# YuliangXiu/ICON

Hardware: AMD Instinct MI355X
Metric: query-points/sec at 256^3 grid (higher is better)
Workload: dtype f32 via 3x f16 split MFMA (22-bit operands, f32 accumulate)

## Files before the change

icon_amd/_lib.py:

```python
from __future__ import annotations

import ctypes as C
import os
import subprocess

_HERE = os.path.dirname(os.path.abspath(__file__))
LIB_PATH = os.environ.get("ICON_AMD_LIB") or os.path.join(_HERE, "libicon_amd.so")
CSRC = os.path.join(_HERE, "csrc")

PRIOR = {"icon": 0, "pamir": 1, "pifu": 2}
CMAP = {"reference": 0, "local": 1}
SEARCH = {"bvh": 0, "brute": 1}
PRECISION = {"f32": 0, "f16x3": 1}

SYMBOLS = [
    "icon_last_error", "icon_version", "icon_device_count",
    "icon_mesh_create", "icon_mesh_destroy", "icon_mesh_vertex_normals", "icon_mesh_stats",
    "icon_mesh_arena_bytes", "icon_mesh_create_arena", "icon_mesh_status", "icon_debug_set_mesh_build", "icon_debug_mesh_layout", "icon_debug_host_mesh_build",
    "icon_sdf_query",
    "icon_feat_create", "icon_feat_destroy", "icon_feat_set_smpl_feats",
    "icon_mlp_create", "icon_mlp_destroy", "icon_mlp_forward", "icon_mlp_set_last_op",
    "icon_work_create", "icon_work_destroy", "icon_work_profile", "icon_work_stage_ms", "icon_work_profile_detail", "icon_work_profile_workgroups", "icon_work_set_steal", "icon_work_set_reserve_cus",
    "icon_query_points", "icon_query_points_dcalib", "icon_query_rows", "icon_grid_rows",
    "icon_volume_any_above", "icon_adaptive_eval", "icon_adaptive_counts", "icon_adaptive_reruns", "icon_grid_eval_slab", "icon_grid_slab_features", "icon_grid_slab_finish", "icon_grid_slab_features_msg",
    "icon_grid_slab_finish_gathered", "icon_debug_set_shell_skip", "icon_debug_set_option", "icon_work_status", "icon_sdf_query_ties", "icon_work_set_tie_rule",
    "icon_export_mesh", "icon_mc_count", "icon_mc_emit", "icon_mc_count_range", "icon_mc_emit_keyed", "icon_debug_traversal_stats", "icon_debug_pair_stats", "icon_debug_walk_stats", "icon_debug_pair_box", "icon_debug_range_box", "icon_debug_box_bound", "icon_debug_box_bound_half", "icon_debug_set_unfused", "icon_debug_mlp_pack_f16x3",
    "icon_visibility", "icon_mesh_components", "icon_clean_mesh", "icon_semantic_voxelize",
    "icon_mesh_batch_create", "icon_mesh_batch_destroy", "icon_mesh_batch_status", "icon_feat_create_batch", "icon_query_points_batch",
    "icon_feat_batch_set_volume", "icon_semantic_voxelize_batch",
    "icon_query_color_bytes", "icon_query_color",
    "icon_render_bytes", "icon_render_normal",
    "icon_silhouette_bytes", "icon_silhouette_forward", "icon_silhouette_backward",
    "icon_render_normal_backward_bytes", "icon_render_normal_backward",
    "icon_render_turntable_bytes", "icon_render_turntable",
    "icon_local_affine_bytes", "icon_local_affine_forward", "icon_local_affine_backward",
    "icon_mesh_priors_bytes", "icon_mesh_priors_forward", "icon_mesh_priors_backward",
    "icon_smpl_bytes", "icon_smpl_forward", "icon_smpl_backward",
    "icon_nearest_vertex", "icon_extract_cloth_bytes", "icon_extract_cloth",
    "icon_normal_consistency_bytes", "icon_normal_consistency",
    "icon_sample_geo_bytes", "icon_sample_geo",
    "icon_train_rows_bytes", "icon_train_rows_forward", "icon_train_rows_backward",
    "icon_train_pamir_forward", "icon_train_vol_bytes", "icon_train_vol_backward",
]

_lib = None


class IconAmdError(RuntimeError):
    pass


def build(force: bool = False) -> str:
    args = ["make", "-j8", "-C", CSRC] + (["-B"] if force else [])
    proc = subprocess.run(args, stdout=subprocess.PIPE, stderr=subprocess.STDOUT, text=True)
    if proc.returncode != 0:
        raise IconAmdError("building libicon_amd.so failed:\n" + proc.stdout[-4000:])
    return LIB_PATH


def lib():
    global _lib
    if _lib is not None:
        return _lib
    if not os.path.exists(LIB_PATH):
        raise IconAmdError(f"{LIB_PATH} not found - run `python -c 'import __graft_entry__ as g; g.build()'` "
                           "or `make -C icon_amd/csrc` (needs hipcc); there is no CPU fallback")
    import torch
    L = C.CDLL(LIB_PATH)
    L.icon_last_error.restype = C.c_char_p
    for name in SYMBOLS:
        if name != "icon_last_error":
            getattr(L, name).restype = C.c_int
    _lib = L
    return L


def check(rc: int, what: str = "") -> None:
    if rc != 0:
        msg = lib().icon_last_error().decode("utf-8", "replace")
        raise IconAmdError(f"{what or 'icon_amd'} failed (code {rc}): {msg}")


def device_count() -> int:
    return int(lib().icon_device_count())


def require_device() -> None:
    if device_count() < 1:
        raise IconAmdError("icon_amd needs a HIP device (MI355X); none is visible and there is no CPU fallback")


def ptr(t) -> C.c_void_p:
    if t is None:
        return C.c_void_p(0)
    if hasattr(t, "data_ptr"):
        assert t.is_contiguous(), "tensor must be contiguous"
        return C.c_void_p(t.data_ptr())
    return C.c_void_p(t.ctypes.data)
```

icon_amd/csrc/common.h:

```cpp
#pragma once
#include <hip/hip_runtime.h>
#include <stdint.h>
#include <functional>
#include <string>
#include <vector>

#include "../../include/icon_amd.h"

namespace icon {
constexpr int kWgRec = 6;
constexpr int kMaxProfGrid = 1024;

void set_error(const std::string &msg);
int fail(int code, const std::string &msg);

#define ICON_HIP(expr)                                                                          \
    do {                                                                                        \
        hipError_t _e = (expr);                                                                 \
        if (_e != hipSuccess)                                                                   \
            return ::icon::fail(ICON_ERR_HIP, std::string(#expr) + ": " + hipGetErrorString(_e)); \
    } while (0)

#define ICON_ARG(cond, msg)                                                  \
    do {                                                                     \
// ... 146 lines not shown
    const float wx[2] = {(float)x1 - ix, ix - (float)t.x0};
    const float wy[2] = {(float)y1 - iy, iy - (float)t.y0};
    const float wz[2] = {(float)z1 - iz, iz - (float)t.z0};
    const bool bx[2] = {t.x0 >= 0 && t.x0 < W, x1 >= 0 && x1 < W};
    const bool by[2] = {t.y0 >= 0 && t.y0 < H, y1 >= 0 && y1 < H};
    const bool bz[2] = {t.z0 >= 0 && t.z0 < D, z1 >= 0 && z1 < D};
#pragma unroll
    for (int k = 0; k < 8; ++k) {
        t.w[k] = (wx[k & 1] * wy[(k >> 1) & 1]) * wz[k >> 2];
        t.in[k] = bx[k & 1] && by[(k >> 1) & 1] && bz[k >> 2];
    }
    t.any = (bx[0] || bx[1]) && (by[0] || by[1]) && (bz[0] || bz[1]);
    return t;
}
__device__ __forceinline__ float trilinear_sample(const TrilinearTaps &t, const float *__restrict__ vol, int H, int W)
{
    float acc = 0.0f;
#pragma unroll
    for (int k = 0; k < 8; ++k) {
        const float v = t.in[k] ? vol[((int64_t)(t.z0 + (k >> 2)) * H + (t.y0 + ((k >> 1) & 1))) * W + (t.x0 + (k & 1))] : 0.0f;
        const float prod = v * t.w[k];
        acc = k == 0 ? prod : acc + prod;
    }
    return acc;
}

struct Calib { float m[12]; const float *d; };

struct Lattice {
    int32_t res, z0, z1;
};

struct LatticeMap {
    int res, z0, nz;
    int tx, ty, tz;
    int remap;
    int off;
    int zs, nzi;
    int sx0, sx1, sy0, sy1;
    int sz0, sz1;
    int trim;
    float trim_need;
    int pk;
};

__device__ __forceinline__ bool not_finite(float y)
{
    uint32_t u = __float_as_uint(y);
    asm volatile("" : "+v"(u));
    return (u & 0x7f800000u) == 0x7f800000u;
}

__device__ __forceinline__ float apply_last_op(float y, int last_op)
{
    return last_op == ICON_LASTOP_SIGMOID ? 1.0f / (1.0f + expf(-y)) : y;
}

struct NearRef { uint16_t *lo; uint8_t *hi; float *d2; const int32_t *map; };

struct SignSrc;

struct BatchDev {
    const MeshDev *meshes;
    const float *calibs;
    int64_t n;
    int64_t plane_stride;
    int B;
    int64_t vol_stride;
};
enum class Src { Lattice, Points, Batch };

}

struct icon_mesh {
    int64_t V = 0, F = 0;
    char *arena = nullptr;
    size_t arena_bytes = 0;
    bool owns_arena = false;
    float *d_vnormals = nullptr;
    icon::MeshDyn *d_dyn = nullptr;
    icon::MeshDyn *h_dyn = nullptr;
    hipEvent_t built = nullptr;
    int depth_bound = 0;
    icon::MeshDev dev{};
};

struct icon_feat {
    float *d_planes = nullptr;
    float *d_vol = nullptr;
    icon::FeatDev dev{};
    int batch = 1;
    int64_t plane_stride = 0;
    int64_t vol_stride = 0;
};

struct icon_mesh_batch {
    int B = 0;
    int64_t V = 0, F = 0;
    int depth_bound = 0;
    std::vector<const icon_mesh *> subj;
    icon::MeshDev *d_table = nullptr;
    icon::MeshDev *h_table = nullptr;
    int *h_status = nullptr;
    hipEvent_t done = nullptr;
};

struct icon_adaptive;
struct icon_mlp {
    int c0 = 0;
    int last_op = 0;
    float *d_blob = nullptr;
    size_t blob_bytes = 0;
    size_t off_w0 = 0, off_b0 = 0, off_w1 = 0, off_b1 = 0, off_w2 = 0, off_w2x = 0, off_b2 = 0, off_w3 = 0;
    size_t off_plain = 0;
    size_t off_flag = 0;
    float b3 = 0.f;
    char *d_f16 = nullptr;
    float f16_inv[3] = {1.f, 1.f, 1.f};
};

namespace icon {
void parallel_for(int n, const std::function<void(int)> &fn);
void debug_sync(const char *what, hipStream_t st);
struct MeshLayout;
int mesh_host_state_get(MeshDyn **h, hipEvent_t *ev);
void mesh_host_state_put(MeshDyn *h, hipEvent_t ev);
void mesh_bind_arena(icon_mesh *m, const MeshLayout &L);
int mesh_build_device(icon_mesh *m, const float *d_verts, const int64_t *d_faces, const float *d_cmap, const float *d_vis, hipStream_t st);
void adaptive_destroy(icon_adaptive *a);
inline int lattice_packet()
{
    static const int pk_env = getenv("ICON_AMD_PACKET") ? atoi(getenv("ICON_AMD_PACKET")) : 0;
    return pk_env == 2 ? 2 : 4;
}
struct McDevState;
void mc_destroy(McDevState *s);
struct CleanState;
void clean_destroy(CleanState *s);
int morton_order(icon_work *w, const float *d_points, const float *calib12, const float *d_calib12, int64_t N, hipStream_t st, const int32_t **perm);
int mlp_launch(const icon_mlp *mlp, const float *d_x, int64_t N, float *d_out, int precision, hipStream_t st);
int mlp_launch_ex(const icon_mlp *mlp, const float *d_x, int64_t N, float *d_out, bool mask, hipStream_t st);
int mlp_rescue_rows(const icon_mlp *mlp, const float *d_x, int64_t N, float *d_out, hipStream_t st);
int mlp_flag_reset(const icon_mlp *mlp, hipStream_t st);
int rescue_always();
int mlp_pack_f16x3(icon_mlp *m, const std::vector<std::vector<float>> &W, const std::vector<std::vector<float>> &B, hipStream_t st);
int mlp_launch_f16x3(const icon_mlp *mlp, const float *d_x, int64_t N, float *d_out, bool mask, hipStream_t st);
uint16_t f32_to_f16_rtn(float f);
float f16_to_f32(uint16_t h);
float pick_scale(const std::vector<float> &W);
int morton_order_batch(icon_work *w, const float *d_points, const float *d_calibs, int64_t n, int B, hipStream_t st, const int32_t **perm);
int ensure_work(icon_work *w, int64_t n_points, bool need_x);
void mark(icon_work *w, int k, hipStream_t st);
bool want_fused(int precision, int search);
int outlier_list(icon_work *w, int64_t N, const int *n_dev, int8_t *signs, bool counted, hipStream_t st);
SignSrc self_signs(const icon_work *work, bool needs);
int resolve_signs(const icon_work *work, SignSrc *sg, hipStream_t st);
int outlier_patch(icon_work *w, int64_t N, int cmap_slot, const SignSrc &sg, hipStream_t st);
int pack_sign_message(const icon_work *w, const int8_t *signs, void *d_msg, int64_t cap, hipStream_t st);
int device_cu_count(int *n_cu);
int once_per_device(int kernel_id, const std::function<hipError_t()> &set);
struct LatticeFast;
struct ShareDbg {
    int *err;
    int ring, lose, spin_log2;
};
int work_share_dbg(icon_work *w, ShareDbg *out);
int work_check_err(icon_work *w);
extern int g_qc_lanes;
extern int g_rn_lanes;
extern int g_tt_chunk;
extern int g_ev_lanes;
enum Opt { kOptPairBox, kOptNodeBox, kOptBoxClamp, kOptLatticeFast, kOptUnfused, kOptShellSkip, kOptMcClassify1, kOptShareWaves, kOptShareRing, kOptShareLose,
           kOptShareSpinLog2, kOptCount };
int option(Opt o);
}

namespace icon {
constexpr float kIdentCalib[12] = {1, 0, 0, 0, 0, 1, 0, 0, 0, 0, 1, 0};
constexpr int kNearLoSlots = 32768;

struct QueryCall {
    const char *who = "";
    Src src = Src::Points;
    const icon_mesh *mesh = nullptr;
    const icon_mesh_batch *mb = nullptr;
    BatchDev bd{};
    const icon_feat *feat = nullptr;
    int prior = 0, cmap_mode = 0, search = 0;
    float sdf_clip = 0.f;
    Calib cal{};
    LatticeMap L{};
    const float *points = nullptr;
    int64_t N = 0;
    const int32_t *map = nullptr;
    const int *n_dev = nullptr;
    int c0 = 0;
    int cmap_slot = 0;
    bool needs_patch = false;
    bool rows_ready = false, patched = false;
};
inline QueryCall query_call(const char *who, Src src, const icon_feat *feat, int prior, float sdf_clip, int cmap_mode, int search)
{
    QueryCall c;
    c.who = who; c.src = src; c.feat = feat; c.prior = prior; c.sdf_clip = sdf_clip; c.cmap_mode = cmap_mode; c.search = search;
    return c;
}
int describe_call(QueryCall &c);
int describe_call(QueryCall &c, const FeatDev &f);
bool coop_search(int64_t N, const icon_work *work);
int call_geometry(QueryCall &c, int8_t *d_signs_out, icon_work *work, hipStream_t st);
int sign_and_list(const QueryCall &c, int8_t *d_signs_out, icon_work *work, hipStream_t st);
int call_finish(QueryCall &c, const icon_mlp *mlp, const SignSrc &fs, float *d_occ, int precision, icon_work *work, hipStream_t st, int za = 0, int zb = 0);
int launch_nearest_batch(const QueryCall &c, icon_work *work, hipStream_t st);
int launch_sign(const QueryCall &c, const icon_work *work, hipStream_t st);
int launch_fused_f16x3(const QueryCall &c, const icon_mlp *mlp, const icon_work *work, int za, int zb, const SignSrc &fs, float *d_occ, hipStream_t st);
int begin_call(icon_work *w, const QueryCall &c, bool need_x = false);
}

struct icon_work {
    float *d_x = nullptr;
    int64_t cap_x = 0;
    uint16_t *d_near16 = nullptr;
    uint8_t *d_near_hi = nullptr;
    float *d_near_d2 = nullptr;
    int64_t cap_points_hi = 0;
    uint8_t *d_code8 = nullptr;
    int64_t cap_points = 0;
    uint64_t *d_grp_mask = nullptr;
    int32_t *d_block_counts = nullptr;
    int64_t *d_block_offsets = nullptr;
    int32_t *d_scan_local = nullptr;
    int64_t *d_scan_part = nullptr;
    int64_t cap_blocks = 0;
    int8_t *d_signs = nullptr;
    int64_t cap_signs = 0;
    int64_t *d_total = nullptr;
    int *d_flag = nullptr;
    mutable bool flag_clean = false;
    int64_t *d_seg = nullptr;
    int32_t *d_row_count = nullptr;
    int32_t *d_row_slots = nullptr;
    int64_t cap_rows = 0;
    int *h_err = nullptr;
    icon::LatticeFast *d_lfast = nullptr;
    uint32_t *d_sort_keys = nullptr;
    int32_t *d_sort_idx = nullptr;
    void *d_sort_tmp = nullptr;
    size_t sort_tmp_bytes = 0;
    int64_t cap_sort = 0;
    icon::QueryCall slab{};
    bool slab_ready = false;
    int tie_rule = 0, tie_ulps = 0;
    int reserve_cus = 0;
    int *h_any = nullptr;
    int *defer_range_flag = nullptr;
    int range_reruns = 0;
    struct icon_adaptive *ad = nullptr;
    icon::McDevState *mc = nullptr;
    icon::CleanState *clean = nullptr;
    bool prof = false;
    hipEvent_t ev[6] = {nullptr, nullptr, nullptr, nullptr, nullptr, nullptr};
    bool ev_search = false;
    unsigned long long *d_clock = nullptr;
    mutable int clock_grid = 0;
    double clock_kernel_ms = 0.0;
    unsigned int *d_steal = nullptr;
    int steal_permille = 150, steal_grp = 2;
    bool ev_valid = false;
};

namespace icon {
inline NearRef work_near(const icon_work *w, const QueryCall &c)
{
    NearRef r;
    r.lo = w->d_near16; r.d2 = w->d_near_d2;
    r.hi = (c.mesh && c.mesh->F > kNearLoSlots) ? w->d_near_hi : nullptr;
    r.map = c.map;
    return r;
}
}
```

icon_amd/csrc/fused_f16x3.hip:

```cpp
#pragma clang fp contract(off)

#include "geom_device.h"
#include "batch_device.h"
#include "mlp_f16x3_device.h"
#include "mlp_plain_device.h"
#include "sign_list_device.h"

#include <algorithm>
#include <mutex>

namespace icon {

constexpr int kTilePts = kF16Pts;
constexpr int kXsOff = kSideOff + 4352;
constexpr int kFusedLds = kXsOff + kTilePts * kXRow * 4;

struct FusedGeom {
    MeshDev m;
    FeatDev f;
    Calib cal;
    int res, z0;
    int off, nx, zs;
    uint32_t nx_magic;
    const float *pts;
    int64_t N;
    const int *n_dev;
    const int32_t *out_map;
    float sdf_clip;
    int cmap_local;
    NearRef near;
    const uint8_t *code8;
    const int64_t *block_offsets;
    const unsigned long long *grp_mask;
    SignSrc sg;
    unsigned long long *clock;
    unsigned int *steal;
    int steal_static, steal_grp, steal_ngrp;
};
constexpr int kPoolOff = kSideOff + kSideFloats * 4;
enum { kPoolNext = 0, kPoolMask, kPoolDone, kPoolPer, kPoolRem, kPoolStatic, kPoolGroup, kPoolNGrp, kPoolGrid, kPoolWords };
static_assert(kPoolOff + 4 * kPoolWords <= kSideOff + 4352, "the draw state lives in the slack behind the side arrays");
constexpr int kPoolLenShift = 24;
constexpr int kMaxStealGroup = 127;

__device__ __forceinline__ void pool_draw(unsigned int *steal, volatile int *pool)
{
    unsigned xcc;
    asm volatile("s_getreg_b32 %0, hwreg(HW_REG_XCC_ID)" : "=s"(xcc));
    const int per = pool[kPoolPer], rem = pool[kPoolRem], stat = pool[kPoolStatic], grp = pool[kPoolGroup], ngrp = pool[kPoolNGrp],
              grid = pool[kPoolGrid];
    int mask = pool[kPoolMask], word = -1;
    for (int s = 0; s < 8 && word < 0; ++s) {
        const int x = (int)((xcc + (unsigned)s) & 7u);
        if ((mask >> x) & 1) continue;
        const int nwg = (grid - x + 7) >> 3;
        for (;;) {
            const int t = (int)atomicAdd(steal + x, 1u);
            if (t >= nwg * ngrp) { mask |= 1 << x; break; }
            const int k = t / ngrp, g = t - k * ngrp, b = x + 8 * k;
            const int sb = b * per + min(b, rem), eb = sb + per + (b < rem ? 1 : 0);
            const int a = sb + stat + g * grp;
            if (a < eb) { word = a | (min(grp, eb - a) << kPoolLenShift); break; }
        }
    }
    pool[kPoolMask] = mask;
    pool[kPoolNext] = word;
}

__device__ __forceinline__ void wg_stamp(unsigned long long *rec)
{
    rec[0] = __builtin_readcyclecounter();
    rec[1] = __builtin_amdgcn_s_memrealtime();
}

static_assert(kScanBlock == 256, "k_sign's 256-point blocks are the blocks of the outlier scan and the tiles of the fused kernel");
template <bool LATTICE>
__global__ __launch_bounds__(256) void k_sign(MeshDev m, Calib cal, int res, int z0, const float *__restrict__ pts, int64_t N,
                                              float sdf_clip, const int32_t *__restrict__ row_count, const int32_t *__restrict__ row_slots,
                                              NearRef near, uint8_t *__restrict__ code8,
                                              int32_t *__restrict__ block_counts, unsigned long long *__restrict__ grp_mask, float far_box2,
                                              const int *__restrict__ n_dev, int *__restrict__ range_flag)
{
    __shared__ int wsum[4];
    if (range_flag && blockIdx.x == 0 && threadIdx.x == 0) *range_flag = 0;
    if (n_dev) { N = *n_dev; if ((int64_t)blockIdx.x * 256 >= N) return; }
    const int64_t i = (int64_t)blockIdx.x * 256 + threadIdx.x;
    const bool live = i < N;
    uint32_t code = 0;
    if (live) {
    f3 p; bool ins;
    if (LATTICE) {
        const int64_t row = i / res;
        const int ix = (int)(i - row * res), iy = (int)(row % res), iz = (int)(row / res);
        p = lattice_world(res, ix, iy, iz + z0);
        ins = inside_row(m, p, row_count, row_slots, row);
    } else {
        p = project(resolve_calib(cal), mk3(pts[3 * i], pts[3 * i + 1], pts[3 * i + 2]));
        ins = inside_bins(m, p);
    }
    const MeshDyn &d = *m.dyn;
    const bool far = box_dist2(d.box_lo[0], d.box_lo[1], d.box_lo[2], d.box_hi[0], d.box_hi[1], d.box_hi[2], p) > far_box2 || near_is_far(near, i);
    code = far ? sign_code_far(p, ins) : sign_code(p, near_d2(near, i), ins, sdf_clip);
    code8[i] = (uint8_t)code;
    }
    const unsigned long long b = __ballot(live && (code & kCodeOutlier));
    if ((threadIdx.x & 63) == 0) {
        wsum[threadIdx.x >> 6] = __popcll(b);
        grp_mask[(int64_t)blockIdx.x * 4 + (threadIdx.x >> 6)] = b;
    }
    __syncthreads();
    if (threadIdx.x == 0) block_counts[blockIdx.x] = wsum[0] + wsum[1] + wsum[2] + wsum[3];
}

template <bool BATCH>
__global__ __launch_bounds__(1024) void k_sign_wide(MeshDev m, Calib cal, const float *__restrict__ pts, int64_t N, float sdf_clip, NearRef near,
                                                    uint8_t *__restrict__ code8, int32_t *__restrict__ block_counts,
                                                    unsigned long long *__restrict__ grp_mask, float far_box2, const int *__restrict__ n_dev,
                                                    int *__restrict__ range_flag, BatchDev bd)
{
    __shared__ unsigned long long gm[4];
    if (range_flag && blockIdx.x == 0 && threadIdx.x == 0) *range_flag = 0;
    if (!BATCH && n_dev) { N = *n_dev; if ((int64_t)blockIdx.x * 256 >= N) return; }
    if (threadIdx.x < 4) gm[threadIdx.x] = 0ull;
    __syncthreads();
    const int s = threadIdx.x & 3, pt = threadIdx.x >> 2;
    const int64_t i = (int64_t)blockIdx.x * 256 + pt;
    const bool live = i < N;
    if (BATCH) {
        const int64_t b = (live ? i : N - 1) / bd.n;
        m = bd.meshes[b]; cal = batch_calib(bd, b);
    }
    uint32_t code = 0;
    const MeshDyn &d = *m.dyn;
    f3 p = mk3(0.f, 0.f, 0.f);
    int beg = 0, end = 0;
    bool brute = false;
    if (live) {
        p = project(resolve_calib(cal), mk3(pts[3 * i], pts[3 * i + 1], pts[3 * i + 2]));
        if (d.gy == 0) brute = true;
        else if (p.y >= d.bin_y0 && p.y <= d.bin_y1 && p.z >= d.bin_z0 && p.z <= d.bin_z1) {
            const int cy = bin_cell(p.y, d.bin_y0, d.bin_inv_y, d.gy);
            const int cz = bin_cell(p.z, d.bin_z0, d.bin_inv_z, d.gz);
            const int cell = cz * d.gy + cy;
            beg = m.bin_start[cell]; end = m.bin_start[cell + 1];
        }
    }
    int cnt = 0;
    for (int k = beg + s; k < end; k += 4) {
        f3 a, b, c; int ia, ib, ic;
        load_tri_full(m.tris + m.bin_slots[k], a, b, c, ia, ib, ic);
        cnt += ray_hit(p, a, b, c, ia, ib, ic);
    }
    cnt += __shfl_xor(cnt, 1);
    cnt += __shfl_xor(cnt, 2);
    if (live) {
        const bool ins = brute ? inside_brute(m, p) : ((cnt & 1) != 0);
        const bool far = box_dist2(d.box_lo[0], d.box_lo[1], d.box_lo[2], d.box_hi[0], d.box_hi[1], d.box_hi[2], p) > far_box2 || near_is_far(near, i);
        code = far ? sign_code_far(p, ins) : sign_code(p, near_d2(near, i), ins, sdf_clip);
        if (s == 0) code8[i] = (uint8_t)code;
    }
    unsigned long long x = __ballot(live && s == 0 && (code & kCodeOutlier));
    x = (x | (x >> 3)) & 0x0303030303030303ull;
    x = (x | (x >> 6)) & 0x000f000f000f000full;
    x = (x | (x >> 12)) & 0x000000ff000000ffull;
    x = (x | (x >> 24)) & 0xffffull;
    const int wave = threadIdx.x >> 6;
    if ((threadIdx.x & 63) == 0 && x) atomicOr(&gm[wave >> 2], x << (16 * (wave & 3)));
    __syncthreads();
    if (threadIdx.x < 4) grp_mask[(int64_t)blockIdx.x * 4 + threadIdx.x] = gm[threadIdx.x];
    if (threadIdx.x == 0) block_counts[blockIdx.x] = __popcll(gm[0]) + __popcll(gm[1]) + __popcll(gm[2]) + __popcll(gm[3]);
}

__global__ __launch_bounds__(256) void k_shell_zero(float *__restrict__ out, int res, int z0, int za, int zb, int row_wgs)
{
    const int planes = zb - za;
    if ((int)blockIdx.x < row_wgs) {
        const int64_t row = (int64_t)blockIdx.x * 256 + threadIdx.x;
        if (row >= (int64_t)planes * res) return;
        const int iy = (int)(row % res), iz = za + (int)(row / res);
        float *o = out + ((int64_t)(iz - z0) * res + iy) * res;
        o[0] = 0.0f; o[res - 1] = 0.0f;
        return;
    }
    const int f = ((int)blockIdx.x - row_wgs) * 4 + (int)(threadIdx.x >> 6);
    const int lane = threadIdx.x & 63;
    int iy, iz;
    if (f < 2 * planes) { iz = za + (f >> 1); iy = (f & 1) ? res - 1 : 0; }
    else {
        const int g = f - 2 * planes;
        const bool has0 = za == 0, has1 = zb == res;
        const int pl = g / res;
        if (pl >= (has0 ? 1 : 0) + (has1 ? 1 : 0)) return;
        iz = (pl == 0 && has0) ? 0 : res - 1;
        iy = g % res;
    }
    float *o = out + ((int64_t)(iz - z0) * res + iy) * res;
    for (int x = lane; x < res; x += 64) o[x] = 0.0f;
}

__device__ __forceinline__ int64_t lattice_item(const FusedGeom &G, int64_t q, int &ix, int &iy, int &iz)
{
    const uint32_t nx = (uint32_t)G.nx, qq = (uint32_t)q;
    const uint32_t r = udiv_fast(qq, nx, G.nx_magic), lx = qq - r * nx, lz = udiv_fast(r, nx, G.nx_magic), ly = r - lz * nx;
    ix = G.off + (int)lx; iy = G.off + (int)ly; iz = G.zs + (int)lz;
    return ((int64_t)(iz - G.z0) * G.res + iy) * G.res + ix;
}

__device__ __forceinline__ int64_t uniform64(int64_t v)
{
    const uint32_t lo = (uint32_t)__builtin_amdgcn_readfirstlane((int)(uint32_t)v);
    const uint32_t hi = (uint32_t)__builtin_amdgcn_readfirstlane((int)(uint32_t)((uint64_t)v >> 32));
    return (int64_t)(((uint64_t)hi << 32) | lo);
}

__device__ __forceinline__ void icon_row(const FusedGeom &G, const MeshDev &m, const FeatDev &f, f3 p, int64_t i, float *xrow, int64_t K, int64_t rank0)
{
    const uint32_t code = G.code8[i];
    Nearest nr;
    nr.slot = near_slot_of(G.near, i); nr.face = 0;
    nr.d2 = (code & kCodeOutlier) ? 0.0f : near_d2(G.near, i);
    const SdfOut o = sdf_attrs(m, p, nr, (code & kCodeInside) != 0);
    float s = o.sdf;
    f3 cmv = o.cm;
    if (code & kCodeOutlier) {
        s = (float)code_sign(code);
        if (G.cmap_local) cmv = mk3(s, s, s);
        else if (K > 0 && (f.smpl_mask & kSmplCmap)) {
            const int64_t blk = i >> 8;
            const int g = (int)(i >> 6) & 3;
            const unsigned long long *mk = G.grp_mask + blk * 4;
            int before = __popcll(mk[g] & ((1ull << (i & 63)) - 1ull));
            if (g > 0) before += __popcll(mk[0]);
            if (g > 1) before += __popcll(mk[1]);
            if (g > 2) before += __popcll(mk[2]);
            const int64_t jr = rank0 + G.block_offsets[blk] + before;
            float c3[3];
            outlier_cmap(G.sg, K, jr, c3);
            cmv = mk3(c3[0], c3[1], c3[2]);
        }
    }
    gather_planes_dyn(f, (f.n_select == 2 && o.vis == 0.0f) ? 1 : 0, p.x, p.y, xrow);
    int hh = f.csel;
    xrow[hh++] = s;
    if (f.smpl_mask & kSmplCmap) { xrow[hh] = cmv.x; xrow[hh + 1] = cmv.y; xrow[hh + 2] = cmv.z; hh += 3; }
    if (f.smpl_mask & kSmplNorm) { xrow[hh] = o.nrm.x; xrow[hh + 1] = o.nrm.y; xrow[hh + 2] = o.nrm.z; }
    xrow[kCodeSlot] = __int_as_float((int)(code & kCodeInCube));
}

template <int PRIOR, Src SRC>
__device__ __forceinline__ void build_row(const FusedGeom &G, const BatchDev &bd, int64_t q, float *xrow, int64_t K, int64_t rank0)
{
    f3 p;
    int64_t i;
    const int64_t b = SRC == Src::Batch ? q / bd.n : 0;
    if (SRC == Src::Lattice) {
        int ix, iy, iz;
        i = lattice_item(G, q, ix, iy, iz);
        p = lattice_world(G.res, ix, iy, iz);
    } else {
        i = q;
        p = project(SRC == Src::Batch ? batch_calib(bd, b) : resolve_calib(G.cal), mk3(G.pts[3 * i], G.pts[3 * i + 1], G.pts[3 * i + 2]));
    }
    const FeatDev f = SRC == Src::Batch ? batch_feat(G.f, bd, b) : G.f;
    if (PRIOR == ICON_PRIOR_ICON) {
// ... 54 lines not shown
            pool[kPoolPer] = per; pool[kPoolRem] = rem; pool[kPoolStatic] = G.steal_static; pool[kPoolGroup] = G.steal_grp;
            pool[kPoolNGrp] = G.steal_ngrp; pool[kPoolGrid] = (int)gridDim.x; pool[kPoolDone] = 0; pool[kPoolMask] = 0; pool[kPoolNext] = -1;
            if (stealing && tile >= tile_end) pool_draw(G.steal, pool);
        }
        __syncthreads();
        if (stealing && tile >= tile_end) {
            const int word = __builtin_amdgcn_readfirstlane(pool[kPoolNext]);
            __syncthreads();
            if (word >= 0) { tile = word & ((1 << kPoolLenShift) - 1); tile_end = tile + (word >> kPoolLenShift); }
        }
    }
    if (tile < tile_end) issue_chunk(w.image, smem, 0, wave0, lane0);

    for (int nb = -1; tile < tile_end;) {
        int tid = threadIdx.x;
        asm volatile("" : "+v"(tid));
        const int lane = tid & 63, wave = __builtin_amdgcn_readfirstlane(tid >> 6);
        const int r = lane & 15, g = lane >> 4;
        const int t = tid;
        const bool draw = !SMALL && stealing && tile + 1 == tile_end;
        if (!SMALL && draw && t == 256) pool_draw(G.steal, pool);
        const bool worker = t < tp;
        int64_t q = (int64_t)tile * tp + (worker ? t : 0);
        if (q >= G.N) q = G.N - 1;
        if (worker) build_row<PRIOR, SRC>(G, bd, q, Xs + t * kXRow, K, rank0);
        __syncthreads();

        nb = (!SMALL && draw) ? __builtin_amdgcn_readfirstlane(pool[kPoolNext]) : -1;
        if (!SMALL && tid == 0) pool[kPoolDone] = pool[kPoolDone] + 1;
        const bool more = tile + 1 < tile_end || nb >= 0;
        if (SMALL && wave >= (tp >> 5)) {
#pragma nounroll
            for (int c = 0; c < 14; c += 2) {
                issue_chunk_units<32>(w.image, smem + kBufBytes, c + 1, wave, lane);
                ICON_CHUNK_BARRIER();
                issue_chunk_units<32>(w.image, smem, c + 2, wave, lane);
                ICON_CHUNK_BARRIER();
            }
            issue_chunk_units<32>(w.image, smem + kBufBytes, 15, wave, lane);
            ICON_CHUNK_BARRIER();
            issue_chunk_units<40>(w.image, smem, 16, wave, lane);
            ICON_CHUNK_BARRIER();
            issue_chunk_units<32>(w.image, smem + kBufBytes, 17, wave, lane);
            ICON_CHUNK_BARRIER();
            issue_chunk_units<32>(w.image, smem, 18, wave, lane);
            ICON_CHUNK_BARRIER();
            issue_chunk_units<32>(w.image, smem + kBufBytes, 19, wave, lane);
            ICON_CHUNK_BARRIER();
            if (more) issue_chunk_units<32>(w.image, smem, 0, wave, lane);
            ++tile;
            continue;
        }
        const int pt = wave * 32 + 16 * (g & 1) + r;
        half8 xb[2];
        const float tail = load_x(Xs + (wave * 32 + r) * kXRow + 8 * (g & 1), Xs + (wave * 32 + 16 + r) * kXRow + 8 * (g & 1), sw3, w.c0, g, xb);
        float maskf = (__float_as_int(Xs[pt * kXRow + kCodeSlot]) & (int)kCodeInCube) ? 1.0f : 0.0f;
        asm volatile("" : "+v"(maskf));

        f32x4 acc1[16][2];
#pragma unroll
        for (int m = 0; m < 16; ++m) acc1[m][0] = acc1[m][1] = *reinterpret_cast<const f32x4 *>(sb1 + m * 16 + 4 * g);
        half8 bh[2], bl[2];
        const LeakyK k0{w.inv0, w.p0, w.q0}, k1{w.inv1, w.p1, w.q1};
        f32x4 acc2[8][2];
        layer01(smem, sb0, w.image, acc1, xb, k0, g, lane, wave, bh, bl);
#pragma unroll
        for (int m2 = 0; m2 < 8; ++m2) acc2[m2][0] = acc2[m2][1] = *reinterpret_cast<const f32x4 *>(sb2 + m2 * 16 + 4 * g);
        activate_split(acc1[0][0], acc1[1][0], acc1[0][1], acc1[1][1], k1, bh, bl);
        l2_chunk<0>(smem, smem + kBufBytes, w.image, acc1, acc2, xb, k1, g, lane, wave, bh, bl);
        ICON_CHUNK_BARRIER();
        l2_chunk<1>(smem + kBufBytes, smem, w.image, acc1, acc2, xb, k1, g, lane, wave, bh, bl);
        ICON_CHUNK_BARRIER();
        l2_chunk<2>(smem, smem + kBufBytes, w.image, acc1, acc2, xb, k1, g, lane, wave, bh, bl);
        ICON_CHUNK_BARRIER();
        l2_chunk<3>(smem + kBufBytes, smem, w.image, acc1, acc2, xb, k1, g, lane, wave, bh, bl, more);

        float y2[2];
        {
            int tid_3 = threadIdx.x;
            asm volatile("" : "+v"(tid_3), "+v"(acc2[0][0]));
            l3_sum(sw3, acc2, tail, LeakyK{w.inv2, w.p2, w.q2}, w.b3, (tid_3 >> 4) & 3, y2);
        }
        int tid_o = threadIdx.x;
        asm volatile("" : "+v"(tid_o), "+v"(y2[0]), "+v"(y2[1]));
        const int g_o = (tid_o >> 4) & 3, pt_o = (tid_o >> 6) * 32 + 16 * (g_o & 1) + (tid_o & 15);
        const float y = apply_last_op(g_o == 0 ? y2[0] : y2[1], w.last_op);
        const int64_t oq = (int64_t)tile * tp + pt_o;
        if (g_o < 2 && oq < G.N) {
            int ix, iy, iz;
            out[SRC == Src::Lattice ? lattice_item(G, oq, ix, iy, iz) : ((SRC == Src::Points && G.out_map) ? (int64_t)G.out_map[oq] : oq)] = masked_result(y, maskf != 0.0f, w.flag);
        }
        if (!SMALL && nb >= 0) {
            tile = nb & ((1 << kPoolLenShift) - 1);
            tile_end = tile + (nb >> kPoolLenShift);
        } else ++tile;
    }
    if (!SMALL && stealing && threadIdx.x == 0) {
        __threadfence();
        if (atomicAdd(G.steal + 8, 1u) == gridDim.x - 1)
            for (int k = 0; k < 9; ++k) atomicExch(G.steal + k, 0u);
    }
    if (G.clock && threadIdx.x == 0 && blockIdx.x < kMaxProfGrid) {
        if (blockIdx.x == 0) wg_stamp(G.clock + 2);
        unsigned long long *rec = G.clock + 4 + kWgRec * blockIdx.x;
        wg_stamp(rec + 2);
        unsigned xcc, hw;
        asm volatile("s_getreg_b32 %0, hwreg(HW_REG_XCC_ID)" : "=s"(xcc));
        asm volatile("s_getreg_b32 %0, hwreg(HW_REG_HW_ID)" : "=s"(hw));
        rec[4] = ((unsigned long long)xcc << 32) | hw;
        rec[5] = SMALL ? 0ull : (unsigned long long)pool[kPoolDone];
    }
}

template <int PRIOR, Src SRC>
__global__ __launch_bounds__(64) void k_rescue_fused(FusedGeom G, float *__restrict__ out, MlpPlain P, const int *flag, int always, BatchDev bd)
{
    __shared__ float s[kPlainLds];
    if (!always && *flag == 0) return;
    if (SRC != Src::Batch && G.n_dev) G.N = *G.n_dev;
    const int lane = threadIdx.x;
    int64_t K = 0, rank0 = 0;
    if (PRIOR == ICON_PRIOR_ICON) launch_sign_extent(G, K, rank0);
    for (int64_t base = (int64_t)blockIdx.x * 64; base < G.N; base += (int64_t)gridDim.x * 64) {
        const int64_t q = base + lane;
        int ix, iy, iz;
        const int64_t o = q < G.N ? (SRC == Src::Lattice ? lattice_item(G, q, ix, iy, iz) : ((SRC == Src::Points && G.out_map) ? (int64_t)G.out_map[q] : q)) : 0;
        const float v = q < G.N ? out[o] : 0.0f;
        unsigned long long todo = __ballot(not_finite(v));
        while (todo) {
            const int b = __ffsll((long long)todo) - 1;
            todo &= todo - 1;
            if (lane == b) {
                float row[kXRow];
#pragma unroll
                for (int k = 0; k < kXRow; ++k) row[k] = 0.0f;
                build_row<PRIOR, SRC>(G, bd, q, row, K, rank0);
#pragma unroll
                for (int k = 0; k < kXRow; ++k) s[k] = k < P.c0 ? row[k] : 0.0f;
            }
            const float y = mlp_plain_wave(P, s, lane);
            if (lane == b) out[o] = y;
            __builtin_amdgcn_wave_barrier();
        }
    }
}

int launch_sign(const QueryCall &c, const icon_work *work, hipStream_t st)
{
    const int64_t N = c.N;
    const int64_t nb = (N + 255) / 256;
    ICON_ARG(nb > 0 && nb < (1ll << 31), "too many workgroups for one launch");
    const float far_box2 = far_box_dist2(c.sdf_clip);
    const NearRef near = work_near(work, c);
    if (c.src == Src::Lattice) hipLaunchKernelGGL(k_sign<true>, dim3((unsigned)nb), dim3(256), 0, st, c.mesh->dev, c.cal, c.L.res, c.L.z0, c.points, N, c.sdf_clip,
                                                  work->d_row_count, work->d_row_slots, near, work->d_code8, work->d_block_counts,
                                                  (unsigned long long *)work->d_grp_mask, far_box2, (const int *)nullptr, work->d_flag);
    else if (c.src == Src::Batch)
        hipLaunchKernelGGL(k_sign_wide<true>, dim3((unsigned)nb), dim3(1024), 0, st, MeshDev{}, Calib{}, c.points, N, c.sdf_clip, near, work->d_code8,
                           work->d_block_counts, (unsigned long long *)work->d_grp_mask, far_box2, (const int *)nullptr, work->d_flag, c.bd);
    else if (c.n_dev || N <= 262144)
        hipLaunchKernelGGL(k_sign_wide<false>, dim3((unsigned)nb), dim3(1024), 0, st, c.mesh->dev, c.cal, c.points, N, c.sdf_clip, near, work->d_code8,
                           work->d_block_counts, (unsigned long long *)work->d_grp_mask, far_box2, c.n_dev, work->d_flag, BatchDev{});
    else hipLaunchKernelGGL(k_sign<false>, dim3((unsigned)nb), dim3(256), 0, st, c.mesh->dev, c.cal, c.L.res, c.L.z0, c.points, N, c.sdf_clip,
                            (const int32_t *)nullptr, (const int32_t *)nullptr, near, work->d_code8, work->d_block_counts,
                            (unsigned long long *)work->d_grp_mask, far_box2, c.n_dev, work->d_flag);
    ICON_HIP(hipGetLastError());
    work->flag_clean = work->d_flag != nullptr;
    return ICON_OK;
}

namespace {
constexpr int kMaxDevices = 64, kMaxKernelIds = 16;
std::mutex g_dev_mutex;
int g_n_cu[kMaxDevices];
bool g_attr_set[kMaxKernelIds][kMaxDevices];
}

int device_cu_count(int *n_cu)
{
    int dev = 0;
    ICON_HIP(hipGetDevice(&dev));
    ICON_ARG(dev >= 0 && dev < kMaxDevices, "device index out of range");
    std::lock_guard<std::mutex> lk(g_dev_mutex);
    if (!g_n_cu[dev]) {
        int n = 0;
        ICON_HIP(hipDeviceGetAttribute(&n, hipDeviceAttributeMultiprocessorCount, dev));
        g_n_cu[dev] = n > 0 ? n : 256;
    }
    *n_cu = g_n_cu[dev];
    return ICON_OK;
}

int once_per_device(int kernel_id, const std::function<hipError_t()> &set)
{
    int dev = 0;
    if (hipGetDevice(&dev) != hipSuccess || dev < 0 || dev >= kMaxDevices || kernel_id < 0 || kernel_id >= kMaxKernelIds) {
        const hipError_t e = set();
        return e == hipSuccess ? ICON_OK : fail(ICON_ERR_HIP, std::string("hipFuncSetAttribute: ") + hipGetErrorString(e));
    }
    std::lock_guard<std::mutex> lk(g_dev_mutex);
    if (g_attr_set[kernel_id][dev]) return ICON_OK;
    const hipError_t e = set();
    if (e != hipSuccess) return fail(ICON_ERR_HIP, std::string("hipFuncSetAttribute: ") + hipGetErrorString(e));
    g_attr_set[kernel_id][dev] = true;
    return ICON_OK;
}

int launch_fused_f16x3(const QueryCall &c, const icon_mlp *mlp, const icon_work *work, int za, int zb, const SignSrc &fs, float *d_occ, hipStream_t st)
{
    const bool lattice = c.src == Src::Lattice;
    const LatticeMap &L = c.L;
    const int prior = c.prior;
    int64_t N = c.N;
    FusedGeom G{};
    if (c.mesh) G.m = c.mesh->dev;
    G.f = c.feat->dev; G.cal = c.cal; G.pts = c.points; G.sdf_clip = c.sdf_clip; G.cmap_local = c.cmap_mode == ICON_CMAP_LOCAL ? 1 : 0;
    if (lattice) {
        const int zs = std::max(za, L.off), ze = std::min(zb, L.res - L.off);
        if (L.off) {
            const int64_t rows = (int64_t)(zb - za) * L.res;
            const int row_wgs = (int)((rows + 255) / 256);
            const int64_t face_rows = 2 * (int64_t)(zb - za) + (int64_t)((za == 0 ? 1 : 0) + (zb == L.res ? 1 : 0)) * L.res;
            if (rows > 0) hipLaunchKernelGGL(k_shell_zero, dim3((unsigned)(row_wgs + (face_rows + 3) / 4)), dim3(256), 0, st, d_occ, L.res, L.z0, za, zb, row_wgs);
        }
        G.res = L.res; G.z0 = L.z0; G.off = L.off; G.nx = L.res - 2 * L.off; G.zs = zs;
        G.nx_magic = udiv_magic((uint32_t)std::max(G.nx, 1));
        N = (ze > zs) ? (int64_t)(ze - zs) * G.nx * G.nx : 0;
    }
    if (N <= 0) { ICON_HIP(hipGetLastError()); return ICON_OK; }
    ICON_ARG(N < (1ll << 31), "fused: more than 2^31 points in one call");
    G.N = N;
    G.near = work_near(work, c); G.code8 = work->d_code8;
    if (!lattice) { G.n_dev = c.n_dev; G.out_map = c.map; }
    G.clock = work->prof ? work->d_clock : nullptr;
    G.steal = nullptr; G.steal_static = 0; G.steal_grp = 1; G.steal_ngrp = 0;
    G.block_offsets = work->d_block_offsets; G.grp_mask = (const unsigned long long *)work->d_grp_mask;
    G.sg = fs;
    int rc = resolve_signs(work, &G.sg, st);
    if (rc) return rc;
    MlpF16Dev w;
    w.image = mlp->d_f16;
    w.side = reinterpret_cast<const float *>(mlp->d_f16 + kImageBytes);
    w.b3 = mlp->b3; w.inv0 = mlp->f16_inv[0]; w.inv1 = mlp->f16_inv[1]; w.inv2 = mlp->f16_inv[2]; w.c0 = mlp->c0; w.last_op = mlp->last_op;
    w.p0 = 0.505f * w.inv0; w.q0 = 0.495f * w.inv0; w.p1 = 0.505f * w.inv1; w.q1 = 0.495f * w.inv1; w.p2 = 0.505f * w.inv2; w.q2 = 0.495f * w.inv2;
    w.flag = work->d_flag ? work->d_flag : reinterpret_cast<int *>(mlp->d_blob + mlp->off_flag);
    const bool defer = work->defer_range_flag != nullptr;
    if (defer) w.flag = work->defer_range_flag;

    int n_cu = 0;
    if ((rc = device_cu_count(&n_cu))) return rc;
    if (defer) {}
    else if (work->d_flag) { if (!work->flag_clean) ICON_HIP(hipMemsetAsync(work->d_flag, 0, sizeof(int), st)); }
    else if ((rc = mlp_flag_reset(mlp, st))) return rc;
    work->flag_clean = false;
    const MlpPlain plain = mlp_plain_of(mlp);
    const int64_t n_resc = std::min<int64_t>((N + 63) / 64, 2048);
    const bool small = prior == ICON_PRIOR_ICON && (c.n_dev != nullptr || N <= 262144);
    const int64_t ntiles = small ? (N + kTilePts / 2 - 1) / (kTilePts / 2) : (N + kTilePts - 1) / kTilePts;
    const unsigned grid = (unsigned)std::min<int64_t>(ntiles, std::max(n_cu - work->reserve_cus, 1));
    {
        const int per = (int)(ntiles / grid);
        const int pool_len = (int)((int64_t)per * work->steal_permille / 1000);
        if (!small && !c.n_dev && work->d_steal && pool_len > 0 && ntiles > (int64_t)grid) {
            G.steal = work->d_steal; G.steal_grp = std::min(work->steal_grp, kMaxStealGroup);
            G.steal_static = per - pool_len;
            G.steal_ngrp = (pool_len + 1 + G.steal_grp - 1) / G.steal_grp;
        }
    }
    if (G.clock) work->clock_grid = (int)std::min<unsigned>(grid, (unsigned)kMaxProfGrid);
    const BatchDev &batch = c.bd;
#define ICON_FUSED(P, S, ID, ...)                                                                                          \
    do {                                                                                                                   \
        if ((rc = once_per_device(ID, [] { return hipFuncSetAttribute(reinterpret_cast<const void *>(k_fused_f16x3<P, Src::S, ##__VA_ARGS__>), \
                                                                    hipFuncAttributeMaxDynamicSharedMemorySize, kFusedLds); }))) return rc; \
        hipLaunchKernelGGL((k_fused_f16x3<P, Src::S, ##__VA_ARGS__>), dim3(grid), dim3(kF16Block), kFusedLds, st, G, d_occ, w, batch); \
        debug_sync("k_fused_f16x3", st);                                                                                   \
        if (!defer) {                                                                                                      \
            hipLaunchKernelGGL((k_rescue_fused<P, Src::S>), dim3((unsigned)n_resc), dim3(64), 0, st, G, d_occ, plain, w.flag, rescue_always(), batch); \
            debug_sync("k_rescue_fused", st);                                                                              \
        }                                                                                                                  \
    } while (0)
    if (c.src == Src::Batch) {
        if (defer || c.n_dev) return fail(ICON_ERR_UNSUPPORTED, "fused: batched call outside point mode");
        if (small) ICON_FUSED(ICON_PRIOR_ICON, Batch, 11, true);
        else if (prior == ICON_PRIOR_ICON) ICON_FUSED(ICON_PRIOR_ICON, Batch, 12);
        else if (prior == ICON_PRIOR_PAMIR) ICON_FUSED(ICON_PRIOR_PAMIR, Batch, 14);
        else ICON_FUSED(ICON_PRIOR_PIFU, Batch, 13);
    }
    else if (small) { if (lattice) ICON_FUSED(ICON_PRIOR_ICON, Lattice, 9, true); else ICON_FUSED(ICON_PRIOR_ICON, Points, 10, true); }
    else if (prior == ICON_PRIOR_ICON) { if (lattice) ICON_FUSED(ICON_PRIOR_ICON, Lattice, 0); else ICON_FUSED(ICON_PRIOR_ICON, Points, 1); }
    else if (prior == ICON_PRIOR_PAMIR) { if (lattice) ICON_FUSED(ICON_PRIOR_PAMIR, Lattice, 2); else ICON_FUSED(ICON_PRIOR_PAMIR, Points, 3); }
    else { if (lattice) ICON_FUSED(ICON_PRIOR_PIFU, Lattice, 4); else ICON_FUSED(ICON_PRIOR_PIFU, Points, 5); }
#undef ICON_FUSED
    ICON_HIP(hipGetLastError());
    return ICON_OK;
}

}
```

icon_amd/csrc/geom_device.h:

```cpp
#pragma once
#pragma clang fp contract(off)

#include "common.h"
#include "mesh_rules.h"

#include <cstdlib>
#include <cstring>

namespace icon {

struct f3 { float x, y, z; };
__device__ __forceinline__ f3 mk3(float x, float y, float z) { f3 r; r.x = x; r.y = y; r.z = z; return r; }
__device__ __forceinline__ f3 sub3(f3 a, f3 b) { return mk3(a.x - b.x, a.y - b.y, a.z - b.z); }
__device__ __forceinline__ float dot3(f3 a, f3 b) { return fmaf(a.z, b.z, fmaf(a.y, b.y, a.x * b.x)); }
__device__ __forceinline__ f3 cross3(f3 a, f3 b)
{
    return mk3(fmaf(a.y, b.z, -(a.z * b.y)), fmaf(a.z, b.x, -(a.x * b.z)), fmaf(a.x, b.y, -(a.y * b.x)));
}

struct TriC {
    f3 a, b, ab, ac, bc;
    float i00, i11, ibc, a00, a01, a11, inn;
};

// ... 730 lines not shown
               fmaf(c2[2], w2, fmaf(c1[2], w1, c0[2] * w0)));
    const float nx = fmaf(n2[0], w2, fmaf(n1[0], w1, n0[0] * w0));
    const float ny = fmaf(n2[1], w2, fmaf(n1[1], w1, n0[1] * w0));
    const float nz = fmaf(n2[2], w2, fmaf(n1[2], w1, n0[2] * w0));
    o.nrm = mk3(-nx, ny, -nz);
    const float vsum = fmaf(s2, w2, fmaf(s1, w1, s0 * w0));
    o.vis = (vsum >= 0.1f) ? 1.0f : 0.0f;
    const float dist = sqrtf(nr.d2) / sqrtf(3.0f);
    o.sdf = inside ? dist : -dist;
    return o;
}

template <int C4>
__device__ __forceinline__ void gather_planes(const FeatDev &f, int sel, float x, float y, float *out )
{
    const int H = f.H, W = f.W;
    const float ix = ((x + 1.0f) / 2.0f) * (float)(W - 1);
    const float iy = ((y + 1.0f) / 2.0f) * (float)(H - 1);
    const float fx = floorf(ix), fy = floorf(iy);
    const int x0 = (int)fx, y0 = (int)fy, x1 = x0 + 1, y1 = y0 + 1;
    const float nw = ((float)x1 - ix) * ((float)y1 - iy);
    const float ne = (ix - (float)x0) * ((float)y1 - iy);
    const float sw = ((float)x1 - ix) * (iy - (float)y0);
    const float se = (ix - (float)x0) * (iy - (float)y0);
    const float4 *base = reinterpret_cast<const float4 *>(f.planes) + (size_t)sel * H * W * C4;
    const bool bx0 = x0 >= 0 && x0 < W, bx1 = x1 >= 0 && x1 < W, by0 = y0 >= 0 && y0 < H, by1 = y1 >= 0 && y1 < H;
    const float4 zero = make_float4(0.f, 0.f, 0.f, 0.f);
#pragma unroll
    for (int c = 0; c < C4; ++c) {
        const float4 t00 = (bx0 && by0) ? base[((size_t)y0 * W + x0) * C4 + c] : zero;
        const float4 t01 = (bx1 && by0) ? base[((size_t)y0 * W + x1) * C4 + c] : zero;
        const float4 t10 = (bx0 && by1) ? base[((size_t)y1 * W + x0) * C4 + c] : zero;
        const float4 t11 = (bx1 && by1) ? base[((size_t)y1 * W + x1) * C4 + c] : zero;
        float acc;
        acc = t00.x * nw; acc += t01.x * ne; acc += t10.x * sw; acc += t11.x * se; out[4 * c + 0] = acc;
        acc = t00.y * nw; acc += t01.y * ne; acc += t10.y * sw; acc += t11.y * se; out[4 * c + 1] = acc;
        acc = t00.z * nw; acc += t01.z * ne; acc += t10.z * sw; acc += t11.z * se; out[4 * c + 2] = acc;
        acc = t00.w * nw; acc += t01.w * ne; acc += t10.w * sw; acc += t11.w * se; out[4 * c + 3] = acc;
    }
}

template <int C4>
__device__ __forceinline__ void gather_volume(const FeatDev &f, float x, float y, float z, float *out )
{
    const int D = f.Dv, H = f.Hv, W = f.Wv;
    const float ix = ((x + 1.0f) / 2.0f) * (float)(W - 1);
    const float iy = ((y + 1.0f) / 2.0f) * (float)(H - 1);
    const float iz = ((z + 1.0f) / 2.0f) * (float)(D - 1);
    const int x0 = (int)floorf(ix), y0 = (int)floorf(iy), z0 = (int)floorf(iz);
    const float tx = ix - (float)x0, ty = iy - (float)y0, tz = iz - (float)z0;
    const float4 *base = reinterpret_cast<const float4 *>(f.vol);
#pragma unroll
    for (int c = 0; c < C4 * 4; ++c) out[c] = 0.0f;
#pragma unroll
    for (int dz = 0; dz < 2; ++dz)
#pragma unroll
        for (int dy = 0; dy < 2; ++dy)
#pragma unroll
            for (int dx = 0; dx < 2; ++dx) {
                const int xi = x0 + dx, yi = y0 + dy, zi = z0 + dz;
                const float wgt = (dx ? tx : 1.0f - tx) * (dy ? ty : 1.0f - ty) * (dz ? tz : 1.0f - tz);
                if (xi >= 0 && xi < W && yi >= 0 && yi < H && zi >= 0 && zi < D) {
#pragma unroll
                    for (int c = 0; c < C4; ++c) {
                        const float4 t = base[(((size_t)zi * H + yi) * W + xi) * C4 + c];
                        out[4 * c + 0] += t.x * wgt; out[4 * c + 1] += t.y * wgt;
                        out[4 * c + 2] += t.z * wgt; out[4 * c + 3] += t.w * wgt;
                    }
                }
            }
}

__device__ __forceinline__ void gather_planes_dyn(const FeatDev &f, int sel, float x, float y, float *out)
{
    switch (f.cpad >> 2) {
        case 1: gather_planes<1>(f, sel, x, y, out); break;
        case 2: gather_planes<2>(f, sel, x, y, out); break;
        case 3: gather_planes<3>(f, sel, x, y, out); break;
        default: gather_planes<4>(f, sel, x, y, out); break;
    }
}


__device__ __forceinline__ int xcd_remap(int b, int nb)
{
    const int q = nb >> 3, r = nb & 7;
    const int xcd = b & 7, k = b >> 3;
    const int start = (xcd < r) ? xcd * (q + 1) : r * (q + 1) + (xcd - r) * q;
    return start + k;
}

__device__ __forceinline__ LatticeMap lattice_trim(LatticeMap L, const MeshDev &m)
{
    if (!L.trim) return L;
    const MeshDyn &d = *m.dyn;
    const int res = L.res, z0 = L.z0, z1 = L.z0 + L.nz;
    int lo[3] = {0, 0, 0}, hi[3] = {res, res, res};
    const float need = L.trim_need;
    if (d.box_lo[0] + 1.0f > need) lo[0] = 1;
    if (1.0f - d.box_hi[0] > need) hi[0] = res - 1;
    if (1.0f - d.box_hi[1] > need) lo[1] = 1;
    if (d.box_lo[1] + 1.0f > need) hi[1] = res - 1;
    if (d.box_lo[2] + 1.0f > need) lo[2] = 1;
    if (1.0f - d.box_hi[2] > need) hi[2] = res - 1;
    L.sx0 = lo[0]; L.sx1 = hi[0]; L.sy0 = lo[1]; L.sy1 = hi[1];
    L.sz0 = max(z0, lo[2]) - z0; L.sz1 = min(z1, hi[2]) - z0;
    if (L.sz1 < L.sz0) L.sz1 = L.sz0;
    const int P = L.pk ? L.pk : 4;
    L.tx = (L.sx1 - L.sx0 + 4 * P - 1) / (4 * P); L.ty = (L.sy1 - L.sy0 + P - 1) / P; L.tz = (L.sz1 - L.sz0 + P - 1) / P;
    L.trim = 0;
    return L;
}

__device__ __forceinline__ bool lattice_point_at(const LatticeMap &L, int t, int wave, int lane, int &ix, int &iy, int &iz)
{
    const int nb = L.tx * L.ty * L.tz;
    if (t >= nb) { ix = iy = iz = 0x3fffffff; return false; }
    if (L.remap == 1) t = xcd_remap(t, nb);
    else if (L.remap == 2) {
        const int full = (nb / (8 * L.tx)) * (8 * L.tx);
        if (t < full) {
            const int r8 = t & 7, k = t >> 3;
            t = ((k / L.tx) * 8 + r8) * L.tx + (k % L.tx);
        }
    }
    const int bty = t / (L.tz * L.tx);
    const int rem = t - bty * (L.tz * L.tx);
    const int btz = rem / L.tx;
    int btx = rem - btz * L.tx;
    if (L.remap == 0) btx = (btx + btz + bty * L.tz) % L.tx;
    const int P = L.pk ? L.pk : 4;
    const bool used = lane < P * P * P;
    const int l = used ? lane : 0;
    ix = L.sx0 + (btx * 4 + wave) * P + l % P;
    iy = L.sy0 + bty * P + (l / P) % P;
    iz = L.sz0 + btz * P + l / (P * P);
    return used && ix < L.sx1 && iy < L.sy1 && iz < L.sz1;
}
__device__ __forceinline__ bool lattice_point(const LatticeMap &L, int &ix, int &iy, int &iz)
{
    return lattice_point_at(L, (int)blockIdx.x, threadIdx.x >> 6, threadIdx.x & 63, ix, iy, iz);
}
struct LatticeFast {
    int32_t sx0, sy0, sz0, sx1, sy1, sz1;
    int32_t tx, tz, txtz, nb;
    uint32_t m_tx, m_txtz;
    int32_t root;
    int32_t pad[3];
};
static_assert(sizeof(LatticeFast) == 64, "LatticeFast layout");
constexpr int kLatticeFastMaxRes = 2048;
constexpr size_t kLatticeFastBytes = sizeof(LatticeFast) + kLatticeFastMaxRes * sizeof(float);
__host__ __device__ inline uint32_t udiv_magic(uint32_t d) { return d > 1 ? (uint32_t)(0x100000000ull / d) : 0xffffffffu; }
__device__ __forceinline__ uint32_t udiv_fast(uint32_t n, uint32_t d, uint32_t m)
{
    const uint32_t q = __umulhi(n, m);
    return q + ((n - q * d >= d) ? 1u : 0u);
}
__device__ __forceinline__ void lattice_fast_write(LatticeFast *out, LatticeMap L, const MeshDev &m)
{
    L = lattice_trim(L, m);
    LatticeFast F;
    F.sx0 = L.sx0; F.sy0 = L.sy0; F.sz0 = L.sz0; F.sx1 = L.sx1; F.sy1 = L.sy1; F.sz1 = L.sz1;
    F.tx = L.tx; F.tz = L.tz; F.txtz = L.tx * L.tz; F.nb = L.tx * L.ty * L.tz;
    F.m_tx = udiv_magic((uint32_t)max(L.tx, 1)); F.m_txtz = udiv_magic((uint32_t)max(L.tx * L.tz, 1));
    F.root = m.dyn->root;
    F.pad[0] = F.pad[1] = F.pad[2] = 0;
    *out = F;
}
__device__ __forceinline__ void lattice_fast_coords(LatticeFast *out, int res, int64_t i)
{
    if (i < res) {
        const float f = (float)(int)i / (float)(res - 1);
        reinterpret_cast<float *>(out + 1)[i] = f * 2.0f + (-1.0f);
    }
}
__device__ __forceinline__ f3 lattice_world_fast(const LatticeFast *lf, int ix, int iy, int iz)
{
    const float *c = reinterpret_cast<const float *>(lf + 1);
    return mk3(c[ix], -c[iy], c[iz]);
}
__device__ __forceinline__ LatticeFast lattice_fast_load(const LatticeFast *lf)
{
    typedef __attribute__((address_space(4))) const int32_t *cint;
    const cint q = (cint)(uintptr_t)lf;
    LatticeFast F;
    F.sx0 = q[0]; F.sy0 = q[1]; F.sz0 = q[2]; F.sx1 = q[3]; F.sy1 = q[4]; F.sz1 = q[5];
    F.tx = q[6]; F.tz = q[7]; F.txtz = q[8]; F.nb = q[9];
    F.m_tx = (uint32_t)q[10]; F.m_txtz = (uint32_t)q[11]; F.root = q[12];
    return F;
}
__device__ __forceinline__ bool lattice_point_fast(const LatticeFast &F, uint32_t t, int wave, int lane, int &cx, int &cy, int &cz)
{
    const uint32_t tx = (uint32_t)F.tx, tz = (uint32_t)F.tz, txtz = (uint32_t)F.txtz;
    const uint32_t bty = udiv_fast(t, txtz, F.m_txtz);
    const uint32_t rem = t - bty * txtz;
    const uint32_t btz = udiv_fast(rem, tx, F.m_tx);
    uint32_t btx = rem - btz * tx;
    const uint32_t rot = btz + bty * tz;
    btx += rot - udiv_fast(rot, tx, F.m_tx) * tx;
    btx = min(btx, btx - tx);
    const int ix = F.sx0 + (int)(btx * 16u) + wave * 4 + (lane & 3);
    const int iy = F.sy0 + (int)(bty * 4u) + ((lane >> 2) & 3);
    const int iz = F.sz0 + (int)(btz * 4u) + (lane >> 4);
    cx = min(ix, F.sx1 - 1); cy = min(iy, F.sy1 - 1); cz = min(iz, F.sz1 - 1);
    return ix < F.sx1 && iy < F.sy1 && iz < F.sz1;
}

__device__ __forceinline__ int packet_center_lane(const LatticeMap &L) { return (L.pk == 0 || L.pk == 4) ? 21 : 0; }

__device__ __forceinline__ void lattice_clamp(const LatticeMap &L, int ix, int iy, int iz, int &cx, int &cy, int &cz)
{
    cx = min(ix, L.sx1 - 1); cy = min(iy, L.sy1 - 1); cz = min(iz, L.sz1 - 1);
}

__device__ __forceinline__ f3 lattice_world(int res, int ix, int iy, int iz)
{
    const float rm1 = (float)(res - 1);
    const float fx = (float)ix / rm1, fy = (float)iy / rm1, fz = (float)iz / rm1;
    return mk3(fx * 2.0f + (-1.0f), fy * (-2.0f) + 1.0f, fz * 2.0f + (-1.0f));
}

struct PacketPoint { bool live; f3 p; int cx, cy, cz; };
__device__ __forceinline__ bool packet_point(LatticeMap L, const MeshDev &m, int tile, int wave, int lane, PacketPoint &out)
{
    L = lattice_trim(L, m);
    if (tile >= L.tx * L.ty * L.tz) return false;
    int ix, iy, iz;
    out.live = lattice_point_at(L, tile, wave, lane, ix, iy, iz);
    lattice_clamp(L, ix, iy, iz, out.cx, out.cy, out.cz);
    out.p = lattice_world(L.res, out.cx, out.cy, out.cz + L.z0);
    return true;
}

constexpr float kFarCoord = 64.0f;
__device__ __forceinline__ f3 clamp_far(f3 r)
{
    r.x = fminf(fmaxf(r.x, -kFarCoord), kFarCoord);
    r.y = fminf(fmaxf(r.y, -kFarCoord), kFarCoord);
    r.z = fminf(fmaxf(r.z, -kFarCoord), kFarCoord);
    return r;
}

__device__ __forceinline__ f3 clamp_raw(f3 r)
{
    constexpr float kBig = 1e18f;
    r.x = fminf(fmaxf(r.x, -kBig), kBig);
    r.y = fminf(fmaxf(r.y, -kBig), kBig);
    r.z = fminf(fmaxf(r.z, -kBig), kBig);
    return r;
}

__device__ __forceinline__ f3 project(const Calib &c, f3 p)
{
    f3 r;
    r.x = fmaf(c.m[2], p.z, fmaf(c.m[1], p.y, c.m[0] * p.x)) + c.m[3];
    r.y = fmaf(c.m[6], p.z, fmaf(c.m[5], p.y, c.m[4] * p.x)) + c.m[7];
    r.z = fmaf(c.m[10], p.z, fmaf(c.m[9], p.y, c.m[8] * p.x)) + c.m[11];
    return clamp_far(r);
}

__device__ __forceinline__ Calib resolve_calib(Calib c)
{
    if (c.d) {
        cfloat *q = as_const(c.d);
#pragma unroll
        for (int k = 0; k < 12; ++k) c.m[k] = q[k];
    }
    return c;
}

__device__ __forceinline__ uint32_t in_cube_bit(f3 p)
{
    const bool in = p.x > -1.0f && p.x < 1.0f && p.y > -1.0f && p.y < 1.0f && p.z > -1.0f && p.z < 1.0f;
    return in ? kCodeInCube : 0u;
}

__device__ __forceinline__ uint32_t sign_code(f3 p, float d2, bool ins, float sdf_clip)
{
    const float dist = sqrtf(d2) / sqrtf(3.0f);
    const float s = ins ? dist : -dist;
    uint32_t code = in_cube_bit(p) | (ins ? kCodeInside : 0u);
    if (fabsf(s) >= sdf_clip) {
        const int sg = (s > 0.0f) ? 1 : ((s < 0.0f) ? -1 : 0);
        code |= kCodeOutlier | ((uint32_t)(sg + 1) << kCodeSignShift);
    }
    return code;
}

constexpr uint32_t kNearFar = 0x8000u;
__device__ __forceinline__ bool near_far_exact(float d2, float sdf_clip)
{
    const float dist = sqrtf(d2) / sqrtf(3.0f);
    return dist >= sdf_clip && dist > 0.0f;
}
__device__ __forceinline__ void store_near(const NearRef &r, int64_t i, const Nearest &nr, float sdf_clip)
{
    const float c2 = sdf_clip * sdf_clip * 3.0f;
    const bool ordinary = sdf_clip > 1e-12f && sdf_clip < 1e12f;
    const bool surely_far = nr.d2 > c2 * 1.0001f, surely_near = nr.d2 < c2 * 0.9999f;
    bool far = surely_far;
    if (__any(!ordinary || !(surely_far || surely_near))) far = near_far_exact(nr.d2, sdf_clip);
    r.lo[i] = (uint16_t)(((uint32_t)nr.slot & 0x7fffu) | (far ? kNearFar : 0u));
    if (r.hi) r.hi[i] = (uint8_t)((uint32_t)nr.slot >> 15);
    if (!far) r.d2[i] = nr.d2;
}
__device__ __forceinline__ int64_t near_index(const NearRef &r, int64_t i) { return r.map ? (int64_t)r.map[i] : i; }
__device__ __forceinline__ bool near_is_far(const NearRef &r, int64_t i) { return (r.lo[near_index(r, i)] & kNearFar) != 0; }
__device__ __forceinline__ float near_d2(const NearRef &r, int64_t i) { return r.d2[near_index(r, i)]; }
__device__ __forceinline__ int near_slot_of(const NearRef &r, int64_t i)
// ... 22 lines not shown
```

icon_amd/csrc/outlier_list.hip:

```cpp
#pragma clang fp contract(off)

#include "sign_list_device.h"
#include "scan_device.h"

#include <algorithm>

namespace icon {

__global__ __launch_bounds__(kScanBlock) void k_outlier_count(const uint8_t *__restrict__ code8, int64_t N, int32_t *block_counts)
{
    __shared__ int wsum[kScanBlock / 64];
    const int64_t i = (int64_t)blockIdx.x * kScanBlock + threadIdx.x;
    const bool o = (i < N) && (code8[i] & kCodeOutlier);
    const unsigned long long b = __ballot(o);
    if ((threadIdx.x & 63) == 0) wsum[threadIdx.x >> 6] = __popcll(b);
    __syncthreads();
    if (threadIdx.x == 0) {
        int s = 0;
        for (int w = 0; w < kScanBlock / 64; ++w) s += wsum[w];
        block_counts[blockIdx.x] = s;
    }
}

__global__ __launch_bounds__(1024) void k_scan_local(const int32_t *__restrict__ counts, int64_t n, int32_t *__restrict__ local, int64_t *__restrict__ part,
                                                     const int *__restrict__ n_points_dev)
{
    __shared__ int64_t wtot[16];
    if (n_points_dev) n = ((int64_t)*n_points_dev + kScanBlock - 1) / kScanBlock;
    const int64_t i = (int64_t)blockIdx.x * 1024 + threadIdx.x;
    const int64_t v = (i < n) ? counts[i] : 0;
    int64_t total;
    const int64_t ex = block_excl_scan<16>(v, wtot, total);
    if (i < n) local[i] = (int32_t)ex;
    if (threadIdx.x == 0) part[blockIdx.x] = total;
}

__global__ __launch_bounds__(1024) void k_scan_apply(const int32_t *__restrict__ local, const int64_t *__restrict__ part, int64_t nchunks, int64_t n,
                                                     int64_t *__restrict__ offsets, int64_t *__restrict__ total, const int *__restrict__ n_points_dev)
{
    __shared__ int64_t wtot[16];
    if (n_points_dev) n = ((int64_t)*n_points_dev + kScanBlock - 1) / kScanBlock;
    int64_t before = 0, all = 0;
    for (int64_t k = threadIdx.x; k < nchunks; k += 1024) { const int64_t t = part[k]; all += t; if (k < blockIdx.x) before += t; }
    int64_t sum_all, sum_before;
    (void)block_excl_scan<16>(all, wtot, sum_all);
    __syncthreads();
    (void)block_excl_scan<16>(before, wtot, sum_before);
    const int64_t i = (int64_t)blockIdx.x * 1024 + threadIdx.x;
    if (i < n) offsets[i] = sum_before + local[i];
    if (blockIdx.x == 0 && threadIdx.x == 0) *total = sum_all;
}

__device__ __forceinline__ int64_t outlier_rank(bool o, const int64_t *block_offsets, int *wsum)
{
    const unsigned long long b = __ballot(o);
    const int lane = threadIdx.x & 63, w = threadIdx.x >> 6;
    if (lane == 0) wsum[w] = __popcll(b);
    __syncthreads();
    int before = 0;
    for (int k = 0; k < w; ++k) before += wsum[k];
    before += __popcll(b & ((1ull << lane) - 1ull));
    return block_offsets[blockIdx.x] + before;
}

__global__ __launch_bounds__(kScanBlock) void k_outlier_compact(const uint8_t *__restrict__ code8, int64_t N,
                                                                const int64_t *block_offsets, int8_t *signs, const int *__restrict__ n_dev)
{
    __shared__ int wsum[kScanBlock / 64];
    if (n_dev) { N = *n_dev; if ((int64_t)blockIdx.x * kScanBlock >= N) return; }
    const int64_t i = (int64_t)blockIdx.x * kScanBlock + threadIdx.x;
    const uint32_t code = (i < N) ? code8[i] : 0u;
    const bool o = code & kCodeOutlier;
    const int64_t r = outlier_rank(o, block_offsets, wsum);
    if (o) signs[r] = (int8_t)code_sign(code);
}

__global__ __launch_bounds__(kScanBlock) void k_outlier_small(const int32_t *__restrict__ counts, const uint8_t *__restrict__ code8, int64_t N,
                                                              int64_t *__restrict__ block_offsets, int64_t *__restrict__ total, int8_t *__restrict__ signs,
                                                              const int *__restrict__ n_dev)
{
    __shared__ int wsum[kScanBlock / 64];
    __shared__ int64_t red[2][kScanBlock / 64];
    if (n_dev) N = *n_dev;
    const int64_t nblk = (N + kScanBlock - 1) / kScanBlock;
    if (blockIdx.x == 0 && threadIdx.x == 0 && nblk == 0) *total = 0;
    if ((int64_t)blockIdx.x >= nblk) return;
    int64_t before = 0, all = 0;
    const bool want_all = blockIdx.x == 0;
    for (int64_t k = threadIdx.x; k < (want_all ? nblk : (int64_t)blockIdx.x); k += kScanBlock) { const int64_t t = counts[k]; all += t; if (k < blockIdx.x) before += t; }
    for (int d = 32; d >= 1; d >>= 1) { before += __shfl_xor(before, d); all += __shfl_xor(all, d); }
    const int lane = threadIdx.x & 63, w = threadIdx.x >> 6;
    if (lane == 0) { red[0][w] = before; red[1][w] = all; }
    __syncthreads();
    before = 0; all = 0;
    for (int k = 0; k < kScanBlock / 64; ++k) { before += red[0][k]; all += red[1][k]; }
    if (threadIdx.x == 0) { block_offsets[blockIdx.x] = before; if (want_all) *total = all; }
    const int64_t i = (int64_t)blockIdx.x * kScanBlock + threadIdx.x;
    const uint32_t code = (i < N) ? code8[i] : 0u;
    const bool o = code & kCodeOutlier;
    const unsigned long long b = __ballot(o);
    if (lane == 0) wsum[w] = __popcll(b);
    __syncthreads();
    int64_t r = before + __popcll(b & ((1ull << lane) - 1ull));
    for (int k = 0; k < w; ++k) r += wsum[k];
    if (o) signs[r] = (int8_t)code_sign(code);
}
constexpr int64_t kSmallListBlocks = 16384;

__global__ __launch_bounds__(kScanBlock) void k_outlier_patch(float *__restrict__ X, const uint8_t *__restrict__ code8, int64_t N, int cmap_slot,
                                                              const int64_t *block_offsets, SignSrc sg)
{
    __shared__ int wsum[kScanBlock / 64];
    int64_t K, rank0;
    sign_list_extent(sg, K, rank0);
    const int64_t i = (int64_t)blockIdx.x * kScanBlock + threadIdx.x;
    const uint32_t code = (i < N) ? code8[i] : 0u;
    const bool o = code & kCodeOutlier;
    const int64_t j = rank0 + outlier_rank(o, block_offsets, wsum);
    if (o && K > 0) {
        float c[3];
        outlier_cmap(sg, K, j, c);
        float *row = X + i * kXRow + cmap_slot;
        row[0] = c[0]; row[1] = c[1]; row[2] = c[2];
    }
}

__global__ __launch_bounds__(256) void k_pack_signs(const int8_t *__restrict__ signs, const int64_t *__restrict__ k_dev, uint8_t *__restrict__ msg, int64_t cap_bytes)
{
    const int64_t K = *k_dev;
    const int64_t t = (int64_t)blockIdx.x * 256 + threadIdx.x;
    if (t == 0) *reinterpret_cast<int64_t *>(msg) = K;
    if (t >= cap_bytes || 4 * t >= K) return;
    uint32_t b = 0;
#pragma unroll
    for (int j = 0; j < 4; ++j)
        if (4 * t + j < K) b |= (uint32_t)(signs[4 * t + j] + 1) << (2 * j);
    msg[8 + t] = (uint8_t)b;
}

__global__ void k_seg_offsets(const int8_t *__restrict__ gathered, int64_t stride, int world, int64_t *__restrict__ seg)
{
    if (threadIdx.x != 0 || blockIdx.x != 0) return;
    int64_t a = 0;
    for (int r = 0; r < world; ++r) { seg[r] = a; a += *reinterpret_cast<const int64_t *>(gathered + (int64_t)r * stride); }
    seg[world] = a;
}

int outlier_list(icon_work *w, int64_t N, const int *n_dev, int8_t *signs, bool counted, hipStream_t st)
{
    const int64_t nblk = (N + kScanBlock - 1) / kScanBlock;
    if (!counted) hipLaunchKernelGGL(k_outlier_count, dim3((unsigned)nblk), dim3(kScanBlock), 0, st, w->d_code8, N, w->d_block_counts);
    const bool one = nblk <= (n_dev ? kSmallListBlocks : 1024);
    if (one) {
        hipLaunchKernelGGL(k_outlier_small, dim3((unsigned)std::max<int64_t>(nblk, 1)), dim3(kScanBlock), 0, st, w->d_block_counts, w->d_code8, N, w->d_block_offsets, w->d_total,
                           signs, n_dev);
    } else {
        const int64_t nchunks = (nblk + 1023) / 1024;
        hipLaunchKernelGGL(k_scan_local, dim3((unsigned)nchunks), dim3(1024), 0, st, w->d_block_counts, nblk, w->d_scan_local, w->d_scan_part, n_dev);
        hipLaunchKernelGGL(k_scan_apply, dim3((unsigned)nchunks), dim3(1024), 0, st, w->d_scan_local, w->d_scan_part, nchunks, nblk, w->d_block_offsets, w->d_total, n_dev);
        hipLaunchKernelGGL(k_outlier_compact, dim3((unsigned)nblk), dim3(kScanBlock), 0, st, w->d_code8, N, w->d_block_offsets, signs, n_dev);
    }
    ICON_HIP(hipGetLastError());
    if (!n_dev) debug_sync(one ? "outlier list (one launch)" : "outlier scan + compact", st);
    return ICON_OK;
}

SignSrc self_signs(const icon_work *work, bool needs)
{
    SignSrc sg{};
    sg.mode = needs ? kSignSelf : kSignNone;
    sg.list = work->d_signs; sg.k_dev = work->d_total;
    return sg;
}

int resolve_signs(const icon_work *work, SignSrc *sg, hipStream_t st)
{
    if (sg->mode != kSignSeg) return ICON_OK;
    if (!work->d_seg) return fail(ICON_ERR_STATE, "sign list: segment offsets buffer missing");
    hipLaunchKernelGGL(k_seg_offsets, dim3(1), dim3(64), 0, st, sg->gathered, sg->stride, sg->world, work->d_seg);
    sg->seg = work->d_seg;
    return ICON_OK;
}

int outlier_patch(icon_work *w, int64_t N, int cmap_slot, const SignSrc &sg, hipStream_t st)
{
    if (sg.mode == kSignNone || (sg.mode == kSignGlobal && sg.k_host <= 0)) return ICON_OK;
    SignSrc s = sg;
    const int rc = resolve_signs(w, &s, st);
    if (rc) return rc;
    const int64_t nblk = (N + kScanBlock - 1) / kScanBlock;
    hipLaunchKernelGGL(k_outlier_patch, dim3((unsigned)nblk), dim3(kScanBlock), 0, st, w->d_x, w->d_code8, N, cmap_slot, w->d_block_offsets, s);
    ICON_HIP(hipGetLastError());
    return ICON_OK;
}

int pack_sign_message(const icon_work *w, const int8_t *signs, void *d_msg, int64_t cap, hipStream_t st)
{
    const int64_t nb = (std::max<int64_t>(cap, 1) + 255) / 256;
    hipLaunchKernelGGL(k_pack_signs, dim3((unsigned)nb), dim3(256), 0, st, signs, w->d_total, (uint8_t *)d_msg, cap);
    ICON_HIP(hipGetLastError());
    return ICON_OK;
}

}
```

icon_amd/csrc/query_kernels.hip:

```cpp
#pragma clang fp contract(off)

#include "query_device.h"
#include "sign_list_device.h"

namespace icon {

template <bool BRUTE>
__global__ __launch_bounds__(kBlock) void k_sdf_query(MeshDev m, const float *__restrict__ pts, int64_t N,
                                                      float *sdf, float *nrm, float *cm, float *vis,
                                                      int64_t *face, uint8_t *inside_out, const int32_t *__restrict__ perm)
{
    __shared__ int lds[kBruteTile * 24];
    int64_t i = (int64_t)blockIdx.x * kBlock + threadIdx.x;
    const bool live = i < N;
    if (live && perm) i = perm[i];
    const int64_t ic = live ? i : (N - 1);
    const f3 p = clamp_raw(mk3(pts[3 * ic], pts[3 * ic + 1], pts[3 * ic + 2]));
    Nearest nr;
    bool ins;
    if (BRUTE) { nr = nearest_brute<kBlock>(m, p, reinterpret_cast<float *>(lds)); ins = inside_brute(m, p); }
    else       { nr = nearest_packet(m, p, live, lds + (threadIdx.x >> 6) * kStackDepth, {mesh_root(m)}); ins = inside_bins(m, p); }
    if (!live) return;
    const SdfOut o = sdf_attrs(m, p, nr, ins);
    sdf[i] = o.sdf;
// ... 136 lines not shown
            f3 a, b, c; int ia, ib, ic;
            load_tri_full(m.tris + slot, a, b, c, ia, ib, ic);
            if (ray_covers(p, a, b, c, ia, ib, ic)) {
                if (n < kRowCap) row_slots[row * kRowCap + n] = slot;
                ++n;
            }
        }
    }
    row_count[row] = (n <= kRowCap) ? n : -1;
}

__global__ __launch_bounds__(kBlock) void k_row_crossings_wide(MeshDev m, LatticeMap L, int32_t *row_count, int32_t *row_slots, LatticeFast *lf)
{
    if (lf && blockIdx.x == 0 && threadIdx.x == 0) lattice_fast_write(lf, L, m);
    if (lf) lattice_fast_coords(lf, L.res, (int64_t)blockIdx.x * kBlock + threadIdx.x);
    const int lane = threadIdx.x & 63, g = lane >> 4, s = lane & 15;
    const int64_t row = ((int64_t)blockIdx.x * kBlock + threadIdx.x) >> 4;
    const bool have = row < (int64_t)L.nz * L.res;
    const MeshDyn &d = *m.dyn;
    if (d.gy == 0) { if (have && s == 0) row_count[row] = -1; return; }
    const int iy = have ? (int)(row % L.res) : 0, iz = have ? (int)(row / L.res) : 0;
    const f3 p = lattice_world(L.res, 0, iy, iz + L.z0);
    int beg = 0, end = 0;
    if (have && p.y >= d.bin_y0 && p.y <= d.bin_y1 && p.z >= d.bin_z0 && p.z <= d.bin_z1) {
        const int cy = bin_cell(p.y, d.bin_y0, d.bin_inv_y, d.gy);
        const int cz = bin_cell(p.z, d.bin_z0, d.bin_inv_z, d.gz);
        const int cell = cz * d.gy + cy;
        beg = m.bin_start[cell]; end = m.bin_start[cell + 1];
    }
    int n = 0;
    for (int k = beg + s; __any(k - s < end); k += 16) {
        bool hit = false;
        int slot = 0;
        if (k < end) {
            slot = m.bin_slots[k];
            f3 a, b, c; int ia, ib, ic;
            load_tri_full(m.tris + slot, a, b, c, ia, ib, ic);
            hit = ray_covers(p, a, b, c, ia, ib, ic);
        }
        const unsigned grp = (unsigned)(__ballot(hit) >> (16 * g)) & 0xffffu;
        const int at = n + __popc(grp & ((1u << s) - 1u));
        if (hit && at < kRowCap) row_slots[row * kRowCap + at] = slot;
        n += __popc(grp);
    }
    if (have && s == 0) row_count[row] = (n <= kRowCap) ? n : -1;
}

bool want_fused(int precision, int search)
{
    return !option(kOptUnfused) && precision == ICON_PRECISION_F16X3 && search != ICON_SEARCH_BRUTE;
}

}

using namespace icon;


extern "C" int icon_sdf_query(const icon_mesh_t *mesh, const float *d_points, int64_t N,
                              float *d_sdf, float *d_norm, float *d_cmap, float *d_vis,
                              int64_t *d_face, uint8_t *d_inside, int search, void *stream)
{
    ICON_ARG(mesh && d_points && d_sdf && d_norm && d_cmap && d_vis, "icon_sdf_query: null argument");
    ICON_ARG(N >= 0, "icon_sdf_query: negative N");
    if (N == 0) return ICON_OK;
    const int64_t nb = (N + kBlock - 1) / kBlock;
    ICON_ARG(nb < (1ll << 31), "icon_sdf_query: N too large for one launch");
    hipStream_t st = (hipStream_t)stream;
    if (search == ICON_SEARCH_BRUTE) {
        hipLaunchKernelGGL(k_sdf_query<true>, dim3((unsigned)nb), dim3(kBlock), 0, st, mesh->dev, d_points, N, d_sdf, d_norm,
                           d_cmap, d_vis, d_face, d_inside, nullptr);
    } else if (N < kPacketMinPoints) {
        const int cap = coop_cap(mesh->depth_bound);
        hipLaunchKernelGGL(k_sdf_query_coop, dim3((unsigned)((N + kCoopWaves - 1) / kCoopWaves)), dim3(kCoopWaves * 64), kCoopWaves * coop_wave_bytes(cap), st,
                           mesh->dev, d_points, N, d_sdf, d_norm, d_cmap, d_vis, d_face, d_inside, cap);
    } else {
        icon_work tmp;
        const int32_t *perm = nullptr;
        int rc = morton_order(&tmp, d_points, kIdentCalib, nullptr, N, st, &perm);
        if (!rc) {
            hipLaunchKernelGGL(k_sdf_query<false>, dim3((unsigned)nb), dim3(kBlock), 0, st, mesh->dev, d_points, N, d_sdf, d_norm,
                               d_cmap, d_vis, d_face, d_inside, perm);
            if (hipGetLastError() != hipSuccess || hipStreamSynchronize(st) != hipSuccess) rc = fail(ICON_ERR_HIP, "icon_sdf_query: launch failed");
        }
        (void)hipFree(tmp.d_sort_keys); (void)hipFree(tmp.d_sort_idx); (void)hipFree(tmp.d_sort_tmp);
        return rc;
    }
    ICON_HIP(hipGetLastError());
    return ICON_OK;
}

namespace icon {

int describe_call(QueryCall &c)
{
    ICON_ARG(c.feat != nullptr, std::string(c.who) + ": feature handle is null");
    if (c.src == Src::Batch) ICON_ARG(c.feat->batch == c.bd.B, std::string(c.who) + ": the feature handle holds another number of subjects");
    return describe_call(c, c.feat->dev);
}

int describe_call(QueryCall &c, const FeatDev &f)
{
    const auto say = [&c](const char *what) { return std::string(c.who) + ": " + what; };
    ICON_ARG(c.prior == ICON_PRIOR_ICON || c.prior == ICON_PRIOR_PAMIR || c.prior == ICON_PRIOR_PIFU, say("unknown prior_type"));
    if (c.prior == ICON_PRIOR_ICON) {
        if (c.src == Src::Batch) {
            ICON_ARG(c.mb != nullptr, say("the icon prior needs a mesh batch"));
            ICON_ARG(c.mb->B == c.bd.B, say("the mesh batch holds another number of subjects"));
            c.mesh = c.mb->subj[0]; c.bd.meshes = c.mb->d_table;
        }
        ICON_ARG(c.mesh != nullptr, say("the icon prior needs a mesh handle"));
        c.c0 = f.csel + 1 + ((f.smpl_mask & kSmplCmap) ? 3 : 0) + ((f.smpl_mask & kSmplNorm) ? 3 : 0);
    } else if (c.prior == ICON_PRIOR_PAMIR) {
        ICON_ARG(f.n_select == 1, say("the pamir prior needs n_select = 1"));
        ICON_ARG(f.vol != nullptr, say("the pamir prior needs a feature handle with a volume (icon_feat_batch_set_volume for a batch)"));
        c.c0 = f.csel + f.Cv;
    } else {
        ICON_ARG(f.n_select == 1, say("the pifu prior needs n_select = 1"));
        c.c0 = f.csel + 1;
    }
    if (c.c0 > kCodeSlot) return fail(ICON_ERR_UNSUPPORTED, say("more than 15 MLP input channels"));
    c.needs_patch = c.prior == ICON_PRIOR_ICON && c.cmap_mode == ICON_CMAP_REFERENCE && (f.smpl_mask & kSmplCmap);
    c.cmap_slot = f.csel + 1;
    return ICON_OK;
}

bool coop_search(int64_t N, const icon_work *work)
{
    static const int mode = getenv("ICON_AMD_POINT_SEARCH") ? atoi(getenv("ICON_AMD_POINT_SEARCH")) : 0;
    return work->tie_rule == 0 && mode != 3 && (N < kPacketMinPoints || mode == 2);
}

namespace {

template <bool LATTICE>
int launch_nearest(const QueryCall &c, icon_work *work, hipStream_t st)
{
    const icon_mesh *mesh = c.mesh;
    const LatticeMap &L = c.L;
    const int64_t N = c.N;
    LatticeFast *lf = nullptr;
    if (LATTICE) {
        const int64_t rows = (int64_t)L.nz * L.res;
        if (rows > work->cap_rows) {
            (void)hipFree(work->d_row_count); (void)hipFree(work->d_row_slots);
            work->d_row_count = nullptr; work->d_row_slots = nullptr; work->cap_rows = 0;
            ICON_HIP(hipMalloc((void **)&work->d_row_count, (size_t)rows * sizeof(int32_t)));
            ICON_HIP(hipMalloc((void **)&work->d_row_slots, (size_t)rows * kRowCap * sizeof(int32_t)));
            work->cap_rows = rows;
        }
        if (option(kOptLatticeFast) && (L.pk == 0 || L.pk == 4) && L.remap == 0 && L.res <= kLatticeFastMaxRes) {
            if (!work->d_lfast) ICON_HIP(hipMalloc((void **)&work->d_lfast, kLatticeFastBytes));
            lf = work->d_lfast;
        }
        if (rows <= 20000)
            hipLaunchKernelGGL(k_row_crossings_wide, dim3((unsigned)((rows * 16 + kBlock - 1) / kBlock)), dim3(kBlock), 0, st, mesh->dev, L,
                               work->d_row_count, work->d_row_slots, lf);
        else
            hipLaunchKernelGGL(k_row_crossings, dim3((unsigned)((rows + kBlock - 1) / kBlock)), dim3(kBlock), 0, st, mesh->dev, L,
                               work->d_row_count, work->d_row_slots, lf);
    }
    int64_t nb;
    if (LATTICE) nb = (int64_t)L.tx * L.ty * L.tz; else nb = (N + kBlock - 1) / kBlock;
    ICON_ARG(nb >= 0 && nb < (1ll << 31), "too many workgroups for one launch");
    const NearRef near = work_near(work, c);
    const int32_t *perm = nullptr;
    const bool alt = work->tie_rule != 0;
    if (!LATTICE && coop_search(N, work)) {
        const int cap = coop_cap(mesh->depth_bound);
        hipLaunchKernelGGL(k_nearest_coop<false>, dim3((unsigned)((N + kCoopWaves - 1) / kCoopWaves)), dim3(kCoopWaves * 64),
                           kCoopWaves * coop_wave_bytes(cap), st, mesh->dev, c.cal, c.points, N, near, cap, c.sdf_clip, BatchDev{});
    } else if (nb > 0) {
        if (!LATTICE) {
            const int rc = morton_order(work, c.points, c.cal.m, c.cal.d, N, st, &perm);
            if (rc) return rc;
        }
        const int share_env = option(kOptShareWaves);
        const int nw = (!LATTICE || alt) ? 1 : ((share_env == 1 || share_env == 8 || share_env == 16) ? share_env : share_waves(nb * 4));
        ShareDbg dbg{};
        if (nw > 1) { const int rc = work_share_dbg(work, &dbg); if (rc) return rc; }
        if (work->prof) (void)hipEventRecord(work->ev[4], st);
        if (nw == 16) hipLaunchKernelGGL(k_nearest_shared<16>, dim3((unsigned)nb * 4), dim3(16 * 64), 0, st, mesh->dev, L, near, c.sdf_clip, dbg);
        else if (nw == 8) hipLaunchKernelGGL(k_nearest_shared<8>, dim3((unsigned)nb * 4), dim3(8 * 64), 0, st, mesh->dev, L, near, c.sdf_clip, dbg);
        else if (alt) hipLaunchKernelGGL((k_nearest<LATTICE, true, false>), dim3((unsigned)nb), dim3(kBlock), 0, st, mesh->dev, c.cal, L, c.points, N, near, perm, c.sdf_clip, work->tie_ulps, lf);
        else if (LATTICE && !(mesh->dev.box_clamp && mesh->dev.pbox_off && mesh->dev.nbox_off)) hipLaunchKernelGGL((k_nearest<true, false, false>), dim3((unsigned)nb), dim3(kBlock), 0, st, mesh->dev, c.cal, L, c.points, N, near, perm, c.sdf_clip, 0, lf);
        else hipLaunchKernelGGL((k_nearest<LATTICE, false, LATTICE>), dim3((unsigned)nb), dim3(kBlock), 0, st, mesh->dev, c.cal, L, c.points, N, near, perm, c.sdf_clip, 0, lf);
        if (work->prof) { (void)hipEventRecord(work->ev[5], st); work->ev_search = true; }
    }
    ICON_HIP(hipGetLastError());
    debug_sync(LATTICE ? "k_row_crossings + k_nearest<lattice>" : "nearest (points)", st);
    return ICON_OK;
}

int feature_rows(QueryCall &c, icon_work *work, hipStream_t st)
{
    if (c.rows_ready) return ICON_OK;
    int rc;
    if ((rc = ensure_work(work, c.N, true))) return rc;
    rc = c.src == Src::Lattice ? launch_features<Src::Lattice>(c, work, st)
       : c.src == Src::Points ? launch_features<Src::Points>(c, work, st) : launch_features<Src::Batch>(c, work, st);
    c.rows_ready = rc == ICON_OK;
    return rc;
}

int materialise_rows(QueryCall &c, icon_work *work, const SignSrc &fs, hipStream_t st)
{
    int rc;
    if ((rc = feature_rows(c, work, st))) return rc;
    if (c.needs_patch && !c.patched) {
        if ((rc = outlier_patch(work, c.N, c.cmap_slot, fs, st))) return rc;
        c.patched = true;
    }
    return ICON_OK;
}

}

int sign_and_list(const QueryCall &c, int8_t *d_signs_out, icon_work *work, hipStream_t st)
{
    int rc;
    if ((rc = launch_sign(c, work, st))) return rc;
    if (!c.n_dev) debug_sync(c.src == Src::Batch ? "k_sign_wide<batch>" : "k_sign", st);
    if (c.needs_patch && (rc = outlier_list(work, c.N, c.n_dev, d_signs_out ? d_signs_out : work->d_signs, true, st))) return rc;
    return ICON_OK;
}

int call_geometry(QueryCall &c, int8_t *d_signs_out, icon_work *work, hipStream_t st)
{
    int rc;
    if (c.prior != ICON_PRIOR_ICON) return ICON_OK;
    if (c.search == ICON_SEARCH_BRUTE) {
        if ((rc = feature_rows(c, work, st))) return rc;
        return c.needs_patch ? outlier_list(work, c.N, nullptr, d_signs_out ? d_signs_out : work->d_signs, false, st) : ICON_OK;
    }
    rc = c.src == Src::Points ? launch_nearest<false>(c, work, st) : c.src == Src::Lattice ? launch_nearest<true>(c, work, st) : launch_nearest_batch(c, work, st);
    if (rc) return rc;
    return sign_and_list(c, d_signs_out, work, st);
}

int call_finish(QueryCall &c, const icon_mlp *mlp, const SignSrc &fs, float *d_occ, int precision, icon_work *work, hipStream_t st, int za, int zb)
{
    int rc;
    const LatticeMap &L = c.L;
    const bool lattice = c.src == Src::Lattice;
    const bool first = !lattice || za == L.z0;
    if (want_fused(precision, c.search)) {
        if (first) mark(work, 2, st);
        rc = launch_fused_f16x3(c, mlp, work, za, zb, fs, d_occ, st);
        mark(work, 3, st);
        return rc;
    }
    if ((rc = materialise_rows(c, work, fs, st))) return rc;
    if (first) mark(work, 2, st);
    if (lattice) {
        const int64_t o = (int64_t)(za - L.z0) * L.res * L.res, n = (int64_t)(zb - za) * L.res * L.res;
        rc = mlp_launch(mlp, work->d_x + o * kXRow, n, d_occ + o, precision, st);
    } else {
        rc = mlp_launch(mlp, work->d_x, c.N, d_occ, precision, st);
    }
    mark(work, 3, st);
    return rc;
}

}

static Calib points_calib(const float *h_calib, const float *d_calib)
{
    Calib cal;
    memcpy(cal.m, h_calib ? h_calib : kIdentCalib, sizeof(cal.m));
    cal.d = d_calib;
    return cal;
}

static int query_points_impl(const icon_mesh_t *mesh, const icon_feat_t *feat, const icon_mlp_t *mlp,
                             int prior_type, float sdf_clip, int cmap_mode, const float *h_calib, const float *d_calib,
                             const float *d_points, int64_t N, float *d_occ,
                             int search, int precision, icon_work_t *work, void *stream)
{
    ICON_ARG(mlp && work && d_points && d_occ, "icon_query_points: null argument");
    ICON_ARG(N >= 0, "icon_query_points: negative N");
    QueryCall c = query_call("icon_query_points", Src::Points, feat, prior_type, sdf_clip, cmap_mode, search);
    c.mesh = mesh; c.cal = points_calib(h_calib, d_calib); c.points = d_points; c.N = N;
    int rc = describe_call(c);
    if (rc) return rc;
    ICON_ARG(c.c0 == mlp->c0, "icon_query_points: MLP input width does not match the feature layout");
    if (N == 0) return ICON_OK;
    hipStream_t st = (hipStream_t)stream;
    if ((rc = begin_call(work, c))) return rc;
    mark(work, 0, st);
    if ((rc = call_geometry(c, nullptr, work, st))) return rc;
    mark(work, 1, st);
    return call_finish(c, mlp, self_signs(work, c.needs_patch), d_occ, precision, work, st);
}

extern "C" int icon_query_points(const icon_mesh_t *mesh, const icon_feat_t *feat, const icon_mlp_t *mlp,
                                 int prior_type, float sdf_clip, int cmap_mode, const float *h_calib,
                                 const float *d_points, int64_t N, float *d_occ,
                                 int search, int precision, icon_work_t *work, void *stream)
{
    return query_points_impl(mesh, feat, mlp, prior_type, sdf_clip, cmap_mode, h_calib, nullptr, d_points, N, d_occ, search,
                             precision, work, stream);
}

extern "C" int icon_query_points_dcalib(const icon_mesh_t *mesh, const icon_feat_t *feat, const icon_mlp_t *mlp,
                                        int prior_type, float sdf_clip, int cmap_mode, const float *d_calib,
                                        const float *d_points, int64_t N, float *d_occ,
                                        int search, int precision, icon_work_t *work, void *stream)
{
    ICON_ARG(d_calib != nullptr, "icon_query_points_dcalib: d_calib is null");
    return query_points_impl(mesh, feat, mlp, prior_type, sdf_clip, cmap_mode, nullptr, d_calib, d_points, N, d_occ, search,
                             precision, work, stream);
}

static int lattice_map(int res, int z0, int z1, const icon_mesh_t *mesh, float sdf_clip, bool shell_ok, LatticeMap *L)
{
    ICON_ARG(res >= 3 && (res & 1) == 1, "lattice resolution must be odd and >= 3 (seg3d_lossless.py:84-86)");
    ICON_ARG(z0 >= 0 && z1 > z0 && z1 <= res, "bad z range");
    L->res = res; L->z0 = z0; L->nz = z1 - z0;
    const int off = (shell_ok && option(kOptShellSkip)) ? 1 : 0;
    L->off = off;
    L->zs = std::max(z0, off); L->nzi = std::min(z1, res - off) - L->zs;
    if (L->nzi < 0) L->nzi = 0;
    L->sx0 = 0; L->sx1 = res; L->sy0 = 0; L->sy1 = res; L->sz0 = 0; L->sz1 = z1 - z0;
    L->pk = lattice_packet();
    L->tx = (L->sx1 - L->sx0 + 4 * L->pk - 1) / (4 * L->pk); L->ty = (L->sy1 - L->sy0 + L->pk - 1) / L->pk; L->tz = (L->sz1 - L->sz0 + L->pk - 1) / L->pk;
    L->trim = (off && mesh) ? 1 : 0;
    L->trim_need = std::sqrt(far_box_dist2(sdf_clip)) * 1.001f + 1e-5f;
    const char *e = getenv("ICON_AMD_XCD_REMAP");
    L->remap = e ? atoi(e) : 0;
    return ICON_OK;
}

static int slab_features_impl(const icon_mesh_t *mesh, const icon_feat_t *feat, int prior_type, float sdf_clip, int cmap_mode,
                              int res, int z0, int z1, int8_t *d_signs_local, int64_t *d_count_local, void *d_msg, int64_t msg_bytes,
                              int search, icon_work_t *work, void *stream)
{
    ICON_ARG(work != nullptr, "icon_grid_slab_features: work is null");
    QueryCall c = query_call("icon_grid_slab_features", Src::Lattice, feat, prior_type, sdf_clip, cmap_mode, search);
    c.mesh = mesh;
    int rc = describe_call(c);
    if (rc) return rc;
    if ((rc = lattice_map(res, z0, z1, prior_type == ICON_PRIOR_ICON ? mesh : nullptr, sdf_clip, search != ICON_SEARCH_BRUTE, &c.L))) return rc;
    hipStream_t st = (hipStream_t)stream;
    const int64_t N = c.N = (int64_t)c.L.nz * res * res;
    ICON_ARG(N < (1ll << 31), "icon_grid_slab_features: more than 2^31 points in one slab");
    if ((rc = begin_call(work, c))) return rc;
    mark(work, 0, st);
    if ((rc = call_geometry(c, d_signs_local, work, st))) return rc;
    if (d_count_local) {
        if (c.needs_patch) ICON_HIP(hipMemcpyAsync(d_count_local, work->d_total, sizeof(int64_t), hipMemcpyDeviceToDevice, st));
        else ICON_HIP(hipMemsetAsync(d_count_local, 0, sizeof(int64_t), st));
    }
    if (d_msg) {
        const int64_t cap = msg_bytes - 8;
        ICON_ARG(msg_bytes >= 8 && cap * 4 >= N, "icon_grid_slab_features_msg: message buffer too small (8 + ceil(points / 4) bytes)");
        if (c.needs_patch) {
            if ((rc = pack_sign_message(work, d_signs_local ? d_signs_local : work->d_signs, d_msg, cap, st))) return rc;
        } else {
            ICON_HIP(hipMemsetAsync(d_msg, 0, sizeof(int64_t), st));
        }
    }
    mark(work, 1, st);
    work->slab = c; work->slab_ready = true;
    return ICON_OK;
}

extern "C" int icon_grid_slab_features(const icon_mesh_t *mesh, const icon_feat_t *feat,
                                       int prior_type, float sdf_clip, int cmap_mode,
                                       int res, int z0, int z1, int8_t *d_signs_local, int64_t *d_count_local,
                                       int search, icon_work_t *work, void *stream)
{
    return slab_features_impl(mesh, feat, prior_type, sdf_clip, cmap_mode, res, z0, z1, d_signs_local, d_count_local, nullptr, 0, search, work, stream);
}

extern "C" int icon_grid_slab_features_msg(const icon_mesh_t *mesh, const icon_feat_t *feat,
                                           int prior_type, float sdf_clip, int cmap_mode,
                                           int res, int z0, int z1, void *d_msg, int64_t msg_bytes,
                                           int search, icon_work_t *work, void *stream)
{
    ICON_ARG(d_msg != nullptr, "icon_grid_slab_features_msg: message buffer is null");
    return slab_features_impl(mesh, feat, prior_type, sdf_clip, cmap_mode, res, z0, z1, nullptr, nullptr, d_msg, msg_bytes, search, work, stream);
}

static QueryCall *prepared_slab(icon_work *work, int res, int z0, int z1)
{
    const LatticeMap &L = work->slab.L;
    return (work->slab_ready && L.res == res && L.z0 == z0 && L.z0 + L.nz == z1) ? &work->slab : nullptr;
}

extern "C" int icon_grid_slab_finish(const icon_mlp_t *mlp, int res, int z0, int z1,
                                     const int8_t *d_signs_global, int64_t k_total, int64_t rank_offset,
                                     float *d_occ, int precision, icon_work_t *work, void *stream)
{
    ICON_ARG(mlp && work && d_occ, "icon_grid_slab_finish: null argument");
    QueryCall *c = prepared_slab(work, res, z0, z1);
    if (!c) return fail(ICON_ERR_STATE, "icon_grid_slab_finish: no matching icon_grid_slab_features call on this workspace");
    ICON_ARG(c->c0 == mlp->c0, "icon_grid_slab_finish: MLP input width does not match the feature layout");
    SignSrc fs{};
    if (c->needs_patch) {
        ICON_ARG(k_total == 0 || d_signs_global != nullptr, "icon_grid_slab_finish: sign list is null");
        fs.mode = kSignGlobal; fs.list = d_signs_global; fs.k_host = k_total; fs.rank_offset = rank_offset;
    }
    work->slab_ready = false;
    return call_finish(*c, mlp, fs, d_occ, precision, work, (hipStream_t)stream, z0, z1);
}

extern "C" int icon_grid_slab_finish_gathered(const icon_mlp_t *mlp, int res, int z0, int z1, int za, int zb,
                                              const void *d_gathered, int64_t stride, int world, int rank,
                                              float *d_occ, int precision, icon_work_t *work, void *stream)
{
    ICON_ARG(mlp && work && d_occ, "icon_grid_slab_finish_gathered: null argument");
    QueryCall *c = prepared_slab(work, res, z0, z1);
    if (!c) return fail(ICON_ERR_STATE, "icon_grid_slab_finish_gathered: no matching icon_grid_slab_features call on this workspace");
    ICON_ARG(za >= z0 && zb > za && zb <= z1, "icon_grid_slab_finish_gathered: planes [za, zb) must lie inside the slab");
    ICON_ARG(c->c0 == mlp->c0, "icon_grid_slab_finish_gathered: MLP input width does not match the feature layout");
    SignSrc fs{};
    if (c->needs_patch) {
        if (d_gathered) {
            ICON_ARG(world >= 1 && world <= kMaxWorld && rank >= 0 && rank < world, "icon_grid_slab_finish_gathered: bad world / rank");
            ICON_ARG(stride >= 8 && (stride & 7) == 0, "icon_grid_slab_finish_gathered: stride must be a multiple of 8 (int64 header)");
            fs.mode = kSignSeg; fs.gathered = (const int8_t *)d_gathered; fs.stride = stride; fs.world = world; fs.rank = rank;
        } else {
            fs = self_signs(work, true);
        }
    }
    return call_finish(*c, mlp, fs, d_occ, precision, work, (hipStream_t)stream, za, zb);
}

static int rows_out(QueryCall &c, float *d_rows, icon_work *work, hipStream_t st)
{
    int rc;
    if ((rc = begin_call(work, c))) return rc;
    if ((rc = call_geometry(c, nullptr, work, st))) return rc;
    if ((rc = materialise_rows(c, work, self_signs(work, c.needs_patch), st))) return rc;
    ICON_HIP(hipMemcpyAsync(d_rows, work->d_x, (size_t)c.N * kXRow * sizeof(float), hipMemcpyDeviceToDevice, st));
    return ICON_OK;
}

extern "C" int icon_query_rows(const icon_mesh_t *mesh, const icon_feat_t *feat, int prior_type, float sdf_clip, int cmap_mode,
                               const float *h_calib, const float *d_calib, const float *d_points, int64_t N, float *d_rows,
                               int search, icon_work_t *work, void *stream)
{
    ICON_ARG(work && d_points && d_rows, "icon_query_rows: null argument");
    ICON_ARG(N >= 0, "icon_query_rows: negative N");
    QueryCall c = query_call("icon_query_rows", Src::Points, feat, prior_type, sdf_clip, cmap_mode, search);
    c.mesh = mesh; c.cal = points_calib(h_calib, d_calib); c.points = d_points; c.N = N;
    const int rc = describe_call(c);
    if (rc) return rc;
    if (N == 0) return ICON_OK;
    return rows_out(c, d_rows, work, (hipStream_t)stream);
}

extern "C" int icon_grid_rows(const icon_mesh_t *mesh, const icon_feat_t *feat, int prior_type, float sdf_clip, int cmap_mode,
                              int res, int z0, int z1, float *d_rows, int search, icon_work_t *work, void *stream)
{
    ICON_ARG(work && d_rows, "icon_grid_rows: null argument");
    QueryCall c = query_call("icon_grid_rows", Src::Lattice, feat, prior_type, sdf_clip, cmap_mode, search);
    c.mesh = mesh;
    int rc = describe_call(c);
    if (rc) return rc;
    if ((rc = lattice_map(res, z0, z1, nullptr, sdf_clip, false, &c.L))) return rc;
    c.N = (int64_t)c.L.nz * res * res;
    ICON_ARG(c.N < (1ll << 31), "icon_grid_rows: more than 2^31 points in one slab");
    return rows_out(c, d_rows, work, (hipStream_t)stream);
}

constexpr int kWalkStatWords = 8;
static int walk_stats(const icon_mesh_t *mesh, int res, int z0, int z1, int clamp, unsigned long long h[kWalkStatWords])
{
    LatticeMap L;
    int rc = lattice_map(res, z0, z1, mesh, 0.05f, true, &L);
    if (rc) return rc;
    unsigned long long *d = nullptr;
    ICON_HIP(hipMalloc((void **)&d, kWalkStatWords * sizeof(unsigned long long)));
    ICON_HIP(hipMemset(d, 0, kWalkStatWords * sizeof(unsigned long long)));
    if (clamp < 0 ? mesh->dev.box_clamp : clamp) hipLaunchKernelGGL(k_walk_stats<true>, dim3((unsigned)(L.tx * L.ty * L.tz)), dim3(kBlock), 0, 0, mesh->dev, L, d);
    else hipLaunchKernelGGL(k_walk_stats<false>, dim3((unsigned)(L.tx * L.ty * L.tz)), dim3(kBlock), 0, 0, mesh->dev, L, d);
    hipError_t e = hipMemcpy(h, d, kWalkStatWords * sizeof(unsigned long long), hipMemcpyDeviceToHost);
    (void)hipFree(d);
    if (e != hipSuccess) return fail(ICON_ERR_HIP, std::string("walk stats: ") + hipGetErrorString(e));
    return ICON_OK;
}
extern "C" int icon_debug_traversal_stats(const icon_mesh_t *mesh, int res, int z0, int z1, uint64_t out[4])
{
    ICON_ARG(mesh && out, "icon_debug_traversal_stats: null argument");
    unsigned long long h[kWalkStatWords];
    int rc = walk_stats(mesh, res, z0, z1, 0, h);
    if (rc) return rc;
    out[0] = h[0]; out[1] = h[1]; out[2] = h[6]; out[3] = h[7];
    return ICON_OK;
}
extern "C" int icon_debug_walk_stats(const icon_mesh_t *mesh, int res, int z0, int z1, uint64_t out[6])
{
    ICON_ARG(mesh && out, "icon_debug_walk_stats: null argument");
    unsigned long long h[kWalkStatWords];
    int rc = walk_stats(mesh, res, z0, z1, -1, h);
    if (rc) return rc;
    for (int k = 0; k < 6; ++k) out[k] = h[k];
    return ICON_OK;
}
extern "C" int icon_debug_pair_stats(const icon_mesh_t *mesh, int res, int z0, int z1, uint64_t out[4])
{
    ICON_ARG(mesh && out, "icon_debug_pair_stats: null argument");
    unsigned long long h[kWalkStatWords];
    int rc = walk_stats(mesh, res, z0, z1, -1, h);
    if (rc) return rc;
    for (int k = 0; k < 4; ++k) out[k] = h[k];
    return ICON_OK;
}

extern "C" int icon_grid_eval_slab(const icon_mesh_t *mesh, const icon_feat_t *feat, const icon_mlp_t *mlp,
                                   int prior_type, float sdf_clip, int cmap_mode,
                                   int res, int z0, int z1, float *d_occ,
                                   int search, int precision, icon_work_t *work, void *stream)
{
    ICON_ARG(mlp && work && d_occ, "icon_grid_eval_slab: null argument");
    int rc = icon_grid_slab_features(mesh, feat, prior_type, sdf_clip, cmap_mode, res, z0, z1, nullptr, nullptr, search, work, stream);
    if (rc) return rc;
    QueryCall &c = work->slab;
    ICON_ARG(c.c0 == mlp->c0, "icon_grid_eval_slab: MLP input width does not match the feature layout");
    work->slab_ready = false;
    return call_finish(c, mlp, self_signs(work, c.needs_patch), d_occ, precision, work, (hipStream_t)stream, z0, z1);
}

extern "C" int icon_sdf_query_ties(const icon_mesh_t *mesh, const float *d_points, int64_t N,
                                   int32_t *d_face, int32_t *d_face2, uint8_t *d_ulps, void *stream)
{
    ICON_ARG(mesh && d_points && d_face && d_face2 && d_ulps, "icon_sdf_query_ties: null argument");
    ICON_ARG(N >= 0, "icon_sdf_query_ties: negative N");
    if (N == 0) return ICON_OK;
    const int64_t nb = (N + kBlock - 1) / kBlock;
    ICON_ARG(nb < (1ll << 31), "icon_sdf_query_ties: N too large for one launch");
    hipStream_t st = (hipStream_t)stream;
    icon_work tmp;
    const int32_t *perm = nullptr;
    int rc = morton_order(&tmp, d_points, kIdentCalib, nullptr, N, st, &perm);
    if (!rc) {
        hipLaunchKernelGGL(k_nearest_ties, dim3((unsigned)nb), dim3(kBlock), 0, st, mesh->dev, d_points, N, perm, d_face, d_face2, d_ulps);
        if (hipGetLastError() != hipSuccess || hipStreamSynchronize(st) != hipSuccess) rc = fail(ICON_ERR_HIP, "icon_sdf_query_ties: launch failed");
    }
    (void)hipFree(tmp.d_sort_keys); (void)hipFree(tmp.d_sort_idx); (void)hipFree(tmp.d_sort_tmp);
    return rc;
}
```

icon_amd/csrc/work.hip:

```cpp
#include "geom_device.h"

#include <algorithm>

namespace icon {
struct Option { Opt id; const char *key, *env; int def; bool (*ok)(int); const char *accepts; };
static constexpr Option kOptions[kOptCount] = {
    {kOptPairBox, "pair_box", "ICON_AMD_PAIR_BOX", 1},
    {kOptNodeBox, "node_box", "ICON_AMD_NODE_BOX", 1},
    {kOptBoxClamp, "box_clamp", "ICON_AMD_BOX_CLAMP", 1},
    {kOptLatticeFast, "lattice_fast", "ICON_AMD_LATTICE_FAST", 1},
    {kOptUnfused, nullptr, "ICON_AMD_UNFUSED", 0},
    {kOptShellSkip, nullptr, "ICON_AMD_SHELL_SKIP", 1},
    {kOptMcClassify1, "mc_classify1", "ICON_AMD_MC_CLASSIFY1", 0},
    {kOptShareWaves, "share_waves", "ICON_AMD_SHARE", -1,
     [](int v) { return v == -1 || v == 1 || v == 4 || v == 8 || v == 16; }, "-1 (by launch size), 1, 4, 8 or 16"},
    {kOptShareRing, "share_ring", nullptr, 0,
     [](int v) { return v == 0 || (v >= 2 && v <= 64 && (v & (v - 1)) == 0); }, "0 or a power of two in 2..64"},
    {kOptShareLose, "share_lose_push", nullptr, 0,
     [](int v) { return v >= 0; }, "a ticket >= 1, or 0"},
    {kOptShareSpinLog2, "share_spin_log2", nullptr, 0,
     [](int v) { return v >= 0 && v < 30; }, "0..29"},
};
constexpr bool options_in_enum_order(int o = 0) { return o == kOptCount || (kOptions[o].id == o && options_in_enum_order(o + 1)); }
static_assert(options_in_enum_order(), "kOptions[] must list the switches in the order of enum Opt");
static int g_opt_value[kOptCount];
static bool g_opt_known[kOptCount];
int option(Opt o)
{
    if (!g_opt_known[o]) {
        const Option &e = kOptions[o];
        const char *v = e.env ? getenv(e.env) : nullptr;
        g_opt_value[o] = !v ? e.def : (e.ok ? atoi(v) : atoi(v) != 0);
        g_opt_known[o] = true;
    }
    return g_opt_value[o];
}
static void set_option(Opt o, int value) { g_opt_value[o] = kOptions[o].ok ? value : (value != 0); g_opt_known[o] = true; }

int work_share_dbg(icon_work *w, ShareDbg *out)
{
    if (!w->h_err) {
        ICON_HIP(hipHostMalloc((void **)&w->h_err, 8 * sizeof(int), hipHostMallocMapped | hipHostMallocPortable));
        memset(w->h_err, 0, 8 * sizeof(int));
    }
    void *dev = nullptr;
    ICON_HIP(hipHostGetDevicePointer(&dev, w->h_err, 0));
    out->err = (int *)dev;
    out->ring = option(kOptShareRing); out->lose = option(kOptShareLose); out->spin_log2 = option(kOptShareSpinLog2);
    return ICON_OK;
}

int work_check_err(icon_work *w)
{
    if (!w || !w->h_err) return ICON_OK;
    volatile int *e = w->h_err;
    const int code = e[0];
    if (code == 0 || code == kShareErrClaimed) return ICON_OK;
    char buf[320];
    static const char *what[] = {"", "a wave waited in vain for the node of its queue ticket (lost or abandoned push)",
                                 "a wave waited in vain for its ring slot to be cleared (ring a full turn behind)",
                                 "an idle wave outlasted its bound while the workgroup was still active"};
    snprintf(buf, sizeof(buf), "shared-walk search: %s [code %d, workgroup %d, wave %d, ticket %d, head %d, tail %d, avail %d, active %d]; the results of "
             "that launch are not to be trusted", what[code >= 1 && code <= 3 ? code : 0], code, e[1], e[7], e[2], e[3], e[4], e[5], e[6]);
    for (int k = 0; k < 8; ++k) e[k] = 0;
    return fail(ICON_ERR_STATE, buf);
}


void mark(icon_work *w, int k, hipStream_t st)
{
    if (w->prof) { (void)hipEventRecord(w->ev[k], st); if (k == 3) w->ev_valid = true; }
}

int ensure_work(icon_work *w, int64_t n_points, bool need_x)
{
    { const int rc = work_check_err(w); if (rc) return rc; }
    if (n_points > w->cap_points) {
        (void)hipFree(w->d_near16); (void)hipFree(w->d_near_d2); w->d_near16 = nullptr; w->d_near_d2 = nullptr; w->cap_points = 0;
        ICON_HIP(hipMalloc((void **)&w->d_near16, (size_t)n_points * sizeof(uint16_t)));
        ICON_HIP(hipMalloc((void **)&w->d_near_d2, (size_t)n_points * sizeof(float)));
        (void)hipFree(w->d_code8); w->d_code8 = nullptr;
        ICON_HIP(hipMalloc((void **)&w->d_code8, (size_t)n_points));
        w->cap_points = n_points;
    }
    if (need_x && n_points > w->cap_x) {
        (void)hipFree(w->d_x); w->d_x = nullptr; w->cap_x = 0;
        ICON_HIP(hipMalloc((void **)&w->d_x, (size_t)n_points * kXRow * sizeof(float)));
        w->cap_x = n_points;
    }
    const int64_t nblk = (n_points + kScanBlock - 1) / kScanBlock;
    if (nblk > w->cap_blocks) {
        (void)hipFree(w->d_block_counts); (void)hipFree(w->d_block_offsets); (void)hipFree(w->d_scan_local); (void)hipFree(w->d_scan_part);
        w->d_block_counts = nullptr; w->d_block_offsets = nullptr; w->d_scan_local = nullptr; w->d_scan_part = nullptr; w->cap_blocks = 0;
        (void)hipFree(w->d_grp_mask); w->d_grp_mask = nullptr;
        ICON_HIP(hipMalloc((void **)&w->d_grp_mask, (size_t)nblk * 4 * sizeof(uint64_t)));
        ICON_HIP(hipMalloc((void **)&w->d_block_counts, (size_t)nblk * sizeof(int32_t)));
        ICON_HIP(hipMalloc((void **)&w->d_block_offsets, (size_t)nblk * sizeof(int64_t)));
        ICON_HIP(hipMalloc((void **)&w->d_scan_local, (size_t)nblk * sizeof(int32_t)));
        ICON_HIP(hipMalloc((void **)&w->d_scan_part, (size_t)((nblk + 1023) / 1024) * sizeof(int64_t)));
        w->cap_blocks = nblk;
    }
    if (n_points > w->cap_signs) {
        (void)hipFree(w->d_signs); w->d_signs = nullptr; w->cap_signs = 0;
        ICON_HIP(hipMalloc((void **)&w->d_signs, (size_t)n_points));
        w->cap_signs = n_points;
    }
    if (!w->d_total) ICON_HIP(hipMalloc((void **)&w->d_total, sizeof(int64_t)));
    if (!w->d_flag) ICON_HIP(hipMalloc((void **)&w->d_flag, sizeof(int)));
    if (!w->d_steal) {
        ICON_HIP(hipMalloc((void **)&w->d_steal, 9 * sizeof(unsigned int)));
        ICON_HIP(hipMemset(w->d_steal, 0, 9 * sizeof(unsigned int)));
    }
    if (!w->d_seg) ICON_HIP(hipMalloc((void **)&w->d_seg, (kMaxWorld + 1) * sizeof(int64_t)));
    return ICON_OK;
}

int begin_call(icon_work *w, const QueryCall &c, bool need_x)
{
    const int rc = ensure_work(w, c.N, need_x);
    if (rc) return rc;
    if (c.prior == ICON_PRIOR_ICON && c.mesh->F > kNearLoSlots && w->cap_points_hi < w->cap_points) {
        (void)hipFree(w->d_near_hi); w->d_near_hi = nullptr; w->cap_points_hi = 0;
        ICON_HIP(hipMalloc((void **)&w->d_near_hi, (size_t)w->cap_points));
        w->cap_points_hi = w->cap_points;
    }
    w->slab_ready = false;
    return ICON_OK;
}

__global__ __launch_bounds__(256) void k_any_above(const float *__restrict__ occ, int res, int sx, int sy, int sz, int nx, int ny, int nz, float level, int *flag)
{
    const int64_t i = (int64_t)blockIdx.x * 256 + threadIdx.x;
    bool pos = false;
    if (i < (int64_t)nx * ny * nz) {
        const int x = (int)(i % nx), y = (int)((i / nx) % ny), z = (int)(i / ((int64_t)nx * ny));
        pos = occ[((int64_t)z * sz * res + (int64_t)y * sy) * res + (int64_t)x * sx] > level;
    }
    if (__any(pos) && (threadIdx.x & 63) == 0) *flag = 1;
}

}

using namespace icon;

extern "C" int icon_work_create(icon_work_t **out)
{
    ICON_ARG(out != nullptr, "icon_work_create: out is null");
    *out = new icon_work();
    return ICON_OK;
}

extern "C" int icon_work_destroy(icon_work_t *w)
{
    if (!w) return ICON_OK;
    (void)hipFree(w->d_x); (void)hipFree(w->d_grp_mask); (void)hipFree(w->d_block_counts); (void)hipFree(w->d_block_offsets); (void)hipFree(w->d_scan_local); (void)hipFree(w->d_scan_part);
    (void)hipFree(w->d_signs); (void)hipFree(w->d_total); (void)hipFree(w->d_flag); (void)hipFree(w->d_seg); (void)hipFree(w->d_row_count); (void)hipFree(w->d_row_slots); (void)hipFree(w->d_lfast); if (w->h_err) (void)hipHostFree(w->h_err); if (w->h_any) (void)hipHostFree(w->h_any); (void)hipFree(w->d_near16); (void)hipFree(w->d_near_hi); (void)hipFree(w->d_near_d2); (void)hipFree(w->d_code8);
    (void)hipFree(w->d_sort_keys); (void)hipFree(w->d_sort_idx); (void)hipFree(w->d_sort_tmp);
    for (int k = 0; k < 6; ++k) if (w->ev[k]) (void)hipEventDestroy(w->ev[k]);
    (void)hipFree(w->d_clock); (void)hipFree(w->d_steal);
    icon::mc_destroy(w->mc);
    icon::clean_destroy(w->clean);
    icon::adaptive_destroy(w->ad);
    delete w;
    return ICON_OK;
}

extern "C" int icon_work_profile_detail(icon_work_t *w, double out[4])
{
    ICON_ARG(w != nullptr && out != nullptr, "icon_work_profile_detail: null argument");
    if (!w->prof || !w->ev_valid) return fail(ICON_ERR_STATE, "icon_work_profile_detail: no profiled call on this workspace");
    ICON_HIP(hipEventSynchronize(w->ev[3]));
    out[0] = out[1] = out[2] = out[3] = 0.0;
    if (w->ev_search) {
        float ms = 0.0f;
        ICON_HIP(hipEventElapsedTime(&ms, w->ev[4], w->ev[5]));
        out[0] = ms;
    }
    unsigned long long c[4] = {0, 0, 0, 0};
    ICON_HIP(hipMemcpy(c, w->d_clock, sizeof(c), hipMemcpyDeviceToHost));
    int dev = 0, khz = 0;
    ICON_HIP(hipGetDevice(&dev));
    ICON_HIP(hipDeviceGetAttribute(&khz, hipDeviceAttributeWallClockRate, dev));
    if (c[2] > c[0] && c[3] > c[1] && khz > 0) {
        out[1] = (double)(c[2] - c[0]);
        out[2] = (double)(c[3] - c[1]) / (double)khz;
        out[3] = out[1] / out[2] * 1e-3;
    }
    return ICON_OK;
}

extern "C" int icon_work_profile_workgroups(icon_work_t *w, double *rec, int cap, int *n)
{
    ICON_ARG(w != nullptr && rec != nullptr && n != nullptr && cap >= 0, "icon_work_profile_workgroups: bad argument");
    if (!w->prof || !w->ev_valid) return fail(ICON_ERR_STATE, "icon_work_profile_workgroups: no profiled call on this workspace");
    ICON_HIP(hipEventSynchronize(w->ev[3]));
    const int g = std::min(w->clock_grid, kMaxProfGrid);
    *n = g;
    if (g <= 0) return ICON_OK;
    std::vector<unsigned long long> c((size_t)kWgRec * g);
    ICON_HIP(hipMemcpy(c.data(), w->d_clock + 4, c.size() * sizeof(unsigned long long), hipMemcpyDeviceToHost));
    int dev = 0, khz = 0;
    ICON_HIP(hipGetDevice(&dev));
    ICON_HIP(hipDeviceGetAttribute(&khz, hipDeviceAttributeWallClockRate, dev));
    ICON_ARG(khz > 0, "icon_work_profile_workgroups: the device reports no wall clock rate");
    unsigned long long t0 = ~0ull;
    for (int b = 0; b < g; ++b) t0 = std::min(t0, c[(size_t)kWgRec * b + 1]);
    for (int b = 0; b < g && b < cap; ++b) {
        const unsigned long long *r = &c[(size_t)kWgRec * b];
        rec[5 * b + 0] = (double)(r[4] >> 32);
        rec[5 * b + 1] = (double)(r[1] - t0) / (double)khz;
        rec[5 * b + 2] = (double)(r[3] - r[1]) / (double)khz;
        rec[5 * b + 3] = (double)(r[2] - r[0]);
        rec[5 * b + 4] = (double)r[5];
    }
    return ICON_OK;
}

extern "C" int icon_work_set_steal(icon_work_t *w, int permille, int group)
{
    ICON_ARG(w != nullptr && permille >= 0 && permille <= 1000 && group >= 1 && group <= 127, "icon_work_set_steal: bad argument");
    w->steal_permille = permille; w->steal_grp = group;
    return ICON_OK;
}

extern "C" int icon_volume_any_above(const float *d_occ, int res, int sx, int sy, int sz, float level, icon_work_t *w, void *stream, int *h_any)
{
    ICON_ARG(d_occ && w && h_any && res >= 1 && sx >= 1 && sy >= 1 && sz >= 1, "icon_volume_any_above: bad argument");
    if (!w->h_any) {
        ICON_HIP(hipHostMalloc((void **)&w->h_any, sizeof(int), hipHostMallocMapped | hipHostMallocPortable));
    }
    void *dev = nullptr;
    ICON_HIP(hipHostGetDevicePointer(&dev, w->h_any, 0));
    *(volatile int *)w->h_any = 0;
    const int nx = (res - 1) / sx + 1, ny = (res - 1) / sy + 1, nz = (res - 1) / sz + 1;
    const int64_t n = (int64_t)nx * ny * nz;
    hipStream_t st = (hipStream_t)stream;
    hipLaunchKernelGGL(icon::k_any_above, dim3((unsigned)((n + 255) / 256)), dim3(256), 0, st, d_occ, res, sx, sy, sz, nx, ny, nz, level, (int *)dev);
    ICON_HIP(hipGetLastError());
    ICON_HIP(hipStreamSynchronize(st));
    *h_any = *(volatile int *)w->h_any;
    return ICON_OK;
}

extern "C" int icon_work_set_reserve_cus(icon_work_t *w, int n)
{
    ICON_ARG(w != nullptr && n >= 0, "icon_work_set_reserve_cus: bad argument");
    w->reserve_cus = n;
    return ICON_OK;
}

extern "C" int icon_work_profile(icon_work_t *w, int enable)
{
    ICON_ARG(w != nullptr, "icon_work_profile: work is null");
    if (enable && !w->ev[0])
        for (int k = 0; k < 6; ++k) ICON_HIP(hipEventCreate(&w->ev[k]));
    if (enable && !w->d_clock) {
        const size_t bytes = (size_t)(4 + kWgRec * kMaxProfGrid) * sizeof(unsigned long long);
        ICON_HIP(hipMalloc((void **)&w->d_clock, bytes));
        ICON_HIP(hipMemset(w->d_clock, 0, bytes));
    }
    w->clock_grid = 0;
    w->ev_search = false;
    w->prof = enable != 0;
    w->ev_valid = false;
    return ICON_OK;
}

extern "C" int icon_work_stage_ms(icon_work_t *w, float out_ms[3])
{
    ICON_ARG(w && out_ms, "icon_work_stage_ms: null argument");
    if (!w->prof || !w->ev_valid) return fail(ICON_ERR_STATE, "icon_work_stage_ms: no profiled call on this workspace");
    ICON_HIP(hipEventSynchronize(w->ev[3]));
    for (int k = 0; k < 3; ++k) ICON_HIP(hipEventElapsedTime(&out_ms[k], w->ev[k], w->ev[k + 1]));
    return ICON_OK;
}

extern "C" int icon_work_status(icon_work_t *work)
{
    ICON_ARG(work != nullptr, "icon_work_status: work is null");
    return work_check_err(work);
}

extern "C" int icon_debug_set_option(const char *key, int value)
{
    ICON_ARG(key != nullptr, "icon_debug_set_option: key is null");
    const std::string k(key);
    for (int o = 0; o < kOptCount; ++o) {
        const Option &e = kOptions[o];
        if (!e.key || k != e.key) continue;
        ICON_ARG(!e.ok || e.ok(value), k + ": " + e.accepts);
        set_option((Opt)o, value);
        return ICON_OK;
    }
    if (k == "qc_lanes") { ICON_ARG(value == 0 || value == 64, "qc_lanes: 0 (default) or 64"); g_qc_lanes = value; }
    else if (k == "rn_lanes") { ICON_ARG(value == 0 || value == 1 || value == 8, "rn_lanes: 0 (default), 1 or 8"); g_rn_lanes = value; }
    else if (k == "tt_chunk") { ICON_ARG(value >= 0 && value <= 32, "tt_chunk: 0 (default) or 1..32"); g_tt_chunk = value; }
    else if (k == "ev_lanes") { ICON_ARG(value == 0 || value == 1 || value == 8, "ev_lanes: 0 (default), 1 or 8"); g_ev_lanes = value; }
    else return fail(ICON_ERR_ARG, "icon_debug_set_option: unknown key " + k);
    return ICON_OK;
}

extern "C" int icon_debug_set_unfused(int on)
{
    set_option(kOptUnfused, on);
    return ICON_OK;
}

extern "C" int icon_debug_set_shell_skip(int on)
{
    set_option(kOptShellSkip, on);
    return ICON_OK;
}

extern "C" int icon_work_set_tie_rule(icon_work_t *work, int rule, int ulps)
{
    ICON_ARG(work != nullptr, "icon_work_set_tie_rule: work is null");
    ICON_ARG(rule == 0 || rule == 1, "icon_work_set_tie_rule: rule must be 0 (definition) or 1 (highest index within ulps)");
    ICON_ARG(ulps >= 0 && ulps <= 255, "icon_work_set_tie_rule: ulps must be 0..255");
    work->tie_rule = rule; work->tie_ulps = ulps;
    return ICON_OK;
}
```

icon_amd/engine.py:

```python
from __future__ import annotations

import contextlib
import ctypes as C
from typing import Optional, Sequence

import numpy as np
import torch
import torch.nn as nn

from . import _lib
from ._lib import IconAmdError, check, ptr
from ._native import need_device, stream as _stream


def _on(t: torch.Tensor):
    return torch.cuda.device(t.device) if t.is_cuda else contextlib.nullcontext()


def _key(*tensors) -> tuple:
    return tuple((t.data_ptr(), t._version, t.shape, t.device) for t in tensors)


def _dev_f32(t: torch.Tensor, what: str) -> torch.Tensor:
    if not t.is_cuda:
# ... 165 lines not shown


class FeatBatchHandle(_Handle):
    _destroy = "icon_feat_destroy"

    def __init__(self, planes: torch.Tensor, n_select: int, smpl_feats: Sequence[str] = ("sdf", "norm", "vis", "cmap"),
                 vol: Optional[torch.Tensor] = None):
        super().__init__()
        _lib.require_device()
        p = _dev_f32(planes, "features")
        if p.dim() != 4:
            raise IconAmdError("features must be [B,C,H,W]")
        B, Cc, H, W = (int(x) for x in p.shape)
        self.B, self.C, self.H, self.W, self.n_select, self.Cv = B, Cc, H, W, n_select, 0
        with _on(p):
            check(_lib.lib().icon_feat_create_batch(ptr(p), C.c_int(B), C.c_int(Cc), C.c_int(H), C.c_int(W), C.c_int(n_select), _stream(),
                                                    C.byref(self.h)), "icon_feat_create_batch")
            if vol is not None:
                v = _dev_f32(vol, "vol_feat")
                if v.dim() != 5:
                    raise IconAmdError(f"vol_feat {tuple(v.shape)} must be [B,Cv,D,H,W]")
                Bv, self.Cv, Dv, Hv, Wv = (int(x) for x in v.shape)
                check(_lib.lib().icon_feat_batch_set_volume(self.h, ptr(v), C.c_int(Bv), C.c_int(self.Cv), C.c_int(Dv), C.c_int(Hv), C.c_int(Wv),
                                                            _stream()), "icon_feat_batch_set_volume")
        if set(smpl_feats) | {"vis"} != {"sdf", "norm", "vis", "cmap"}:
            check(_lib.lib().icon_feat_set_smpl_feats(self.h, C.c_int(int("cmap" in smpl_feats)), C.c_int(int("norm" in smpl_feats))),
                  "icon_feat_set_smpl_feats")


class FeatHandle(FeatBatchHandle):

    def __init__(self, planes: torch.Tensor, n_select: int, vol: Optional[torch.Tensor] = None,
                 smpl_feats: Sequence[str] = ("sdf", "norm", "vis", "cmap")):
        if planes.dim() == 4 and planes.shape[0] != 1:
            raise IconAmdError("batch size must be 1 (lib/common/seg3d_lossless.py:73)")
        if vol is not None:
            vol = vol[:1] if vol.dim() == 5 else vol[None]
        super().__init__(planes if planes.dim() == 4 else planes[None], n_select, smpl_feats, vol)


def _np32(t) -> np.ndarray:
    if isinstance(t, torch.Tensor):
        t = t.detach().to("cpu", torch.float32).numpy()
    return np.ascontiguousarray(t, dtype=np.float32)


def effective_filters(state_dict: dict) -> dict:
    if not any(k.endswith("weight_g") for k in state_dict):
        return state_dict
    out = {k: v for k, v in state_dict.items() if not (k.endswith("weight_g") or k.endswith("weight_v"))}
    for k, g in state_dict.items():
        if k.endswith("weight_g"):
            v = state_dict[k[:-1] + "v"]
            g, v = (torch.as_tensor(t).detach().float().cpu() for t in (g, v))
            out[k[:-2]] = torch._weight_norm(v, g, 0)
    return out


class MlpHandle(_Handle):
    _destroy = "icon_mlp_destroy"

    def __init__(self, state_dict, res_layers: Sequence[int] = (2, 3, 4), bn_eps: float = 1e-5, last_op: Optional[str] = None):
        super().__init__()
        if last_op not in (None, "sigmoid"):
            raise IconAmdError(f"unsupported last_op {last_op!r} (None or 'sigmoid')")
        _lib.require_device()
        state_dict = effective_filters(state_dict)
        n = 0
        while f"filters.{n}.weight" in state_dict:
            n += 1
        if n == 0:
            raise IconAmdError("state_dict has no filters.0.weight")
        W = [_np32(state_dict[f"filters.{l}.weight"]) for l in range(n)]
        W = [w.reshape(w.shape[0], -1) for w in W]
        b = [_np32(state_dict[f"filters.{l}.bias"]) for l in range(n)]
        has_bn = f"norms.0.running_mean" in state_dict
        cin = (C.c_int * n)(*[w.shape[1] for w in W])
        cout = (C.c_int * n)(*[w.shape[0] for w in W])
        is_res = (C.c_int * n)(*[1 if l in tuple(res_layers) else 0 for l in range(n)])
        self.c0 = int(W[0].shape[1])

        def parr(arrs):
            return (C.c_void_p * len(arrs))(*[a.ctypes.data for a in arrs])

        keep = [W, b]
        if has_bn:
            bn = [[_np32(state_dict[f"norms.{l}.{k}"]) for l in range(n - 1)]
                  for k in ("weight", "bias", "running_mean", "running_var")]
            keep.append(bn)
            bn_ptrs = [parr(x) for x in bn]
        else:
            bn_ptrs = [None] * 4
        check(_lib.lib().icon_mlp_create(C.c_int(n), cin, cout, is_res, parr(W), parr(b), bn_ptrs[0], bn_ptrs[1],
                                         bn_ptrs[2], bn_ptrs[3], C.c_float(bn_eps), _stream(), C.byref(self.h)),
              "icon_mlp_create")
        self.last_op = last_op
        if last_op == "sigmoid":
            check(_lib.lib().icon_mlp_set_last_op(self.h, C.c_int(1)), "icon_mlp_set_last_op")

    def forward(self, x: torch.Tensor, precision: str = "f16x3") -> torch.Tensor:
        x = _dev_f32(x, "x")
        if x.dim() != 2 or x.shape[1] != 16:
            raise IconAmdError("x must be [N,16]")
        out = torch.empty(x.shape[0], dtype=torch.float32, device=x.device)
        check(_lib.lib().icon_mlp_forward(self.h, ptr(x), C.c_int64(x.shape[0]), ptr(out),
                                          C.c_int(_lib.PRECISION[precision]), _stream()), "icon_mlp_forward")
        return out



_WARNED_VOXELIZER = False
_WARNED_COMPOSED = set()


class Workspace(_Handle):
    _destroy = "icon_work_destroy"

    def __init__(self):
        super().__init__()
        check(_lib.lib().icon_work_create(C.byref(self.h)), "icon_work_create")

    def set_tie_rule(self, rule: int, ulps: int = 0) -> None:
        check(_lib.lib().icon_work_set_tie_rule(self.h, C.c_int(rule), C.c_int(ulps)), "icon_work_set_tie_rule")

    def status(self) -> None:
        check(_lib.lib().icon_work_status(self.h), "icon_work_status")

    def set_reserve_cus(self, n: int) -> None:
        check(_lib.lib().icon_work_set_reserve_cus(self.h, C.c_int(int(n))), "icon_work_set_reserve_cus")

    def profile(self, enable: bool = True) -> None:
        check(_lib.lib().icon_work_profile(self.h, C.c_int(int(enable))), "icon_work_profile")

    def profile_detail(self) -> dict:
        out = (C.c_double * 4)()
        check(_lib.lib().icon_work_profile_detail(self.h, out), "icon_work_profile_detail")
        return {"nearest_ms": float(out[0]), "fused_cycles": float(out[1]), "fused_wall_ms": float(out[2]), "effective_clock_mhz": float(out[3])}

    def profile_workgroups(self):
        import numpy as np
        cap = 1024
        out = (C.c_double * (5 * cap))()
        n = C.c_int(0)
        check(_lib.lib().icon_work_profile_workgroups(self.h, out, C.c_int(cap), C.byref(n)), "icon_work_profile_workgroups")
        return np.frombuffer(out, dtype=np.float64)[:5 * min(n.value, cap)].reshape(-1, 5).copy()

    def set_steal(self, permille: int, group: int = 2) -> None:
        check(_lib.lib().icon_work_set_steal(self.h, C.c_int(int(permille)), C.c_int(int(group))), "icon_work_set_steal")

    def adaptive_reruns(self) -> int:
        n = C.c_int(0)
        check(_lib.lib().icon_adaptive_reruns(self.h, C.byref(n)), "icon_adaptive_reruns")
        return int(n.value)

    def stage_ms(self):
        out = (C.c_float * 3)()
        check(_lib.lib().icon_work_stage_ms(self.h, out), "icon_work_stage_ms")
        return float(out[0]), float(out[1]), float(out[2])


def check_regressor(regressor, norm_mlp: Optional[str] = None) -> None:
    if isinstance(regressor, dict):
        if any(k.startswith("norms.") for k in regressor) and "norms.0.running_mean" not in regressor and norm_mlp not in ("group", "instance"):
            raise IconAmdError("regressor state_dict has norms.* without running statistics (GroupNorm / affine InstanceNorm): set "
                               "engine.norm_mlp = 'group' or 'instance' - a state_dict does not say which")
        return
    norm = getattr(regressor, "norm", "batch")
    has_norm_layers = len(getattr(regressor, "norms", ())) > 0
    if has_norm_layers and norm not in ("batch", "group", "instance"):
        raise IconAmdError(f"if_regressor.norm = {norm!r} with norm layers: lib/net/MLP.py builds norm layers for 'batch', "
                           "'group' and 'instance' only")
    lo = getattr(regressor, "last_op", None)
    if lo is not None and not isinstance(lo, nn.Sigmoid):
        raise IconAmdError(f"if_regressor.last_op = {type(lo).__name__}: only None (cfg.test_mode) and nn.Sigmoid "
                           "(lib/net/HGPIFuNet.py:133) are evaluated")
    if getattr(regressor, "training", False) and norm == "batch":
        raise IconAmdError("if_regressor is in training mode: BatchNorm batch statistics cannot be folded - call .eval()")


def regressor_last_op(regressor) -> Optional[str]:
    return "sigmoid" if isinstance(getattr(regressor, "last_op", None), nn.Sigmoid) else None


def regressor_state_dict(regressor, norm_mlp: Optional[str] = None) -> dict:
    check_regressor(regressor, norm_mlp)
    if isinstance(regressor, dict):
        return regressor
    return {k: v for k, v in regressor.state_dict().items() if "num_batches_tracked" not in k}


def _device_of(*cands):
    for c in cands:
        if isinstance(c, (list, tuple)) and c:
            c = c[-1]
        if isinstance(c, torch.Tensor) and c.is_cuda:
            return c
    return None


def _guarded(fn):
    import functools

    @functools.wraps(fn)
    def wrapper(self, *args, **kw):
        t = _device_of(*args, *kw.values())
        if t is None:
            return fn(self, *args, **kw)
        with _on(t):
            return fn(self, *args, **kw)
    return wrapper


class IconQueryEngine:

    def __init__(self, prior_type: str = "icon", sdf_clip: float = 0.05,
                 smpl_feats: Sequence[str] = ("sdf", "norm", "vis", "cmap"),
                 cmap_mode: str = "reference", search: str = "bvh", precision: str = "f16x3",
                 res_layers: Sequence[int] = (2, 3, 4), voxelizer: str = "auto"):
        if prior_type not in _lib.PRIOR:
            raise IconAmdError(f"unknown prior_type {prior_type!r}")
        if prior_type == "icon":
            unknown = set(smpl_feats) - {"sdf", "norm", "vis", "cmap"}
            if unknown:
                raise IconAmdError(f"smpl_feats = {list(smpl_feats)}: only sdf / norm / vis / cmap exist")
        self.smpl_feats = tuple(smpl_feats)
        self.prior_type, self.sdf_clip = prior_type, float(sdf_clip)
        self.cmap_mode, self.search, self.precision = cmap_mode, search, precision
        self.res_layers = tuple(res_layers)
        if voxelizer not in ("auto", "hip", "reference"):
            raise IconAmdError("voxelizer must be 'auto', 'hip' or 'reference'")
        self.voxelizer = voxelizer
        self.last_op = None
        self.tie_rule = None
        self.norm_mlp = None
        self._calibrated = None
        self._work_tie = None
        self.netG = None
        self.work = None
        self._mesh = self._mesh_key = self._mesh_src = None
        self._feat = self._feat_key = self._feat_src = None
        self._mlp = self._mlp_key = self._mlp_src = None
        self._vol = self._vol_key = self._vol_src = None
        self._vol_cached = None
        self._volb_key = self._volb_src = self._volb_cached = None
        self._smpl_feat_dict = None
        self._regressor = None

    @classmethod
    def attach(cls, netG, **kw) -> "IconQueryEngine":
        import sys
        mod = sys.modules.get(type(netG).__module__)
        if mod is not None and getattr(mod, "maskout", False):
            raise IconAmdError(f"attach: {type(netG).__module__}.maskout is set (lib/net/HGPIFuNet.py:32,337-342 overwrites the sdf "
                               "channel of points without image features with it); the HIP query evaluates the shipped maskout = False path only")
        eng = cls(prior_type=netG.prior_type, sdf_clip=netG.sdf_clip,
                  smpl_feats=getattr(netG, "smpl_feats", ("sdf", "norm", "vis", "cmap")),
                  res_layers=getattr(netG.if_regressor, "res_layers", (2, 3, 4)), **kw)
        eng.netG = netG
        netG.query = eng.query
        netG.icon_amd_engine = eng
        return eng

    def set_mesh(self, smpl_verts, smpl_faces, smpl_cmap, smpl_vis) -> None:
        self._smpl_feat_dict = dict(smpl_verts=smpl_verts, smpl_faces=smpl_faces, smpl_cmap=smpl_cmap,
                                    smpl_vis=smpl_vis)

    def set_regressor(self, regressor) -> None:
        self._regressor = regressor

    def set_volume_features(self, vol_feat: torch.Tensor) -> None:
        self._vol = vol_feat

    split_features = True

    def _work(self, i: int = 0) -> Workspace:
        if i == 0:
            if self.work is None:
                self.work = Workspace()
                self._work_tie = None
            w = self.work
        else:
            extra = self.__dict__.setdefault("_extra_works", {})
            if i not in extra:
                extra[i] = Workspace()
                extra[i]._tie = None
            w = extra[i]
        have = self._work_tie if i == 0 else w._tie
        if self.tie_rule != have:
            if self.tie_rule is None:
                w.set_tie_rule(0, 0)
            else:
                kind, ulps = self.tie_rule
                if kind != "highest":
                    raise IconAmdError("tie_rule must be None or ('highest', ulps)")
                w.set_tie_rule(1, int(ulps))
            if i == 0:
                self._work_tie = self.tie_rule
            else:
                w._tie = self.tie_rule
        return w

    def _mesh_handle(self) -> Optional[MeshHandle]:
        if self.prior_type != "icon":
            return None
        d = self.netG.smpl_feat_dict if self.netG is not None else self._smpl_feat_dict
        if d is None:
# ... 570 lines not shown
```

include/icon_amd.h:

```cpp
#ifndef ICON_AMD_H
#define ICON_AMD_H

#include <stdint.h>

#ifdef __cplusplus
extern "C" {
#endif

#define ICON_AMD_VERSION 100

enum {
    ICON_OK = 0,
    ICON_ERR_ARG = 1,
    ICON_ERR_HIP = 2,
    ICON_ERR_UNSUPPORTED = 3,
    ICON_ERR_STATE = 4
};

enum { ICON_PRIOR_ICON = 0, ICON_PRIOR_PAMIR = 1, ICON_PRIOR_PIFU = 2 };

enum { ICON_CMAP_REFERENCE = 0, ICON_CMAP_LOCAL = 1 };

enum { ICON_PRECISION_F32 = 0, ICON_PRECISION_F16X3 = 1 };

enum { ICON_SEARCH_BVH = 0, ICON_SEARCH_BRUTE = 1 };


typedef struct icon_mesh icon_mesh_t;
typedef struct icon_feat icon_feat_t;
typedef struct icon_mlp  icon_mlp_t;
typedef struct icon_work icon_work_t;

const char *icon_last_error(void);
int icon_version(void);
int icon_device_count(void);

int icon_mesh_create(const float *d_verts, int64_t V, const int64_t *d_faces, int64_t F,
                     const float *d_cmap, const float *d_vis, void *stream, icon_mesh_t **out);
int icon_mesh_arena_bytes(int64_t V, int64_t F, int64_t *bytes);
int icon_mesh_create_arena(const float *d_verts, int64_t V, const int64_t *d_faces, int64_t F,
                           const float *d_cmap, const float *d_vis, void *d_arena, int64_t arena_bytes,
                           void *stream, icon_mesh_t **out);
int icon_mesh_destroy(icon_mesh_t *mesh);
int icon_mesh_status(const icon_mesh_t *mesh, int wait, int *bits);
int icon_mesh_vertex_normals(const icon_mesh_t *mesh, float *d_out, void *stream);
int icon_mesh_stats(const icon_mesh_t *mesh, int64_t out[6]);

int icon_sdf_query(const icon_mesh_t *mesh, const float *d_points, int64_t N,
                   float *d_sdf, float *d_norm, float *d_cmap, float *d_vis,
                   int64_t *d_face, uint8_t *d_inside, int search, void *stream);

int icon_feat_create(const float *d_planes, int C, int H, int W, int n_select,
                     const float *d_vol, int Cv, int Dv, int Hv, int Wv,
                     void *stream, icon_feat_t **out);
int icon_feat_destroy(icon_feat_t *feat);
int icon_feat_set_smpl_feats(icon_feat_t *feat, int has_cmap, int has_norm);

int icon_mlp_create(int n_layers, const int *cin, const int *cout, const int *is_res,
                    const float *const *h_W, const float *const *h_b,
                    const float *const *h_bn_gamma, const float *const *h_bn_beta,
                    const float *const *h_bn_mean, const float *const *h_bn_var,
                    float bn_eps, void *stream, icon_mlp_t **out);
int icon_mlp_destroy(icon_mlp_t *mlp);
enum { ICON_LASTOP_NONE = 0, ICON_LASTOP_SIGMOID = 1 };
int icon_mlp_set_last_op(icon_mlp_t *mlp, int last_op);
int icon_mlp_forward(const icon_mlp_t *mlp, const float *d_x, int64_t N, float *d_out,
                     int precision, void *stream);

int icon_work_create(icon_work_t **out);
int icon_work_destroy(icon_work_t *work);
int icon_work_profile(icon_work_t *work, int enable);
int icon_work_set_reserve_cus(icon_work_t *work, int n);
int icon_work_stage_ms(icon_work_t *work, float out_ms[3]);
int icon_work_profile_detail(icon_work_t *work, double out[4]);
int icon_work_profile_workgroups(icon_work_t *work, double *rec, int cap, int *n);
int icon_work_set_steal(icon_work_t *work, int permille, int group);

int icon_query_points(const icon_mesh_t *mesh, const icon_feat_t *feat, const icon_mlp_t *mlp,
                      int prior_type, float sdf_clip, int cmap_mode, const float *h_calib,
                      const float *d_points, int64_t N, float *d_occ,
                      int search, int precision, icon_work_t *work, void *stream);

int icon_query_points_dcalib(const icon_mesh_t *mesh, const icon_feat_t *feat, const icon_mlp_t *mlp,
                             int prior_type, float sdf_clip, int cmap_mode, const float *d_calib,
                             const float *d_points, int64_t N, float *d_occ,
                             int search, int precision, icon_work_t *work, void *stream);

typedef struct icon_mesh_batch icon_mesh_batch_t;
int icon_mesh_batch_create(const icon_mesh_t *const *meshes, int B, void *stream, icon_mesh_batch_t **out);
int icon_mesh_batch_destroy(icon_mesh_batch_t *mb);
#define ICON_MESH_BATCH_FACES_DIFFER 0x10
int icon_mesh_batch_status(const icon_mesh_batch_t *mb, int wait, int *bits);

int icon_feat_create_batch(const float *d_planes, int B, int C, int H, int W, int n_select, void *stream, icon_feat_t **out);

int icon_feat_batch_set_volume(icon_feat_t *feat, const float *d_vol, int B, int Cv, int Dv, int Hv, int Wv, void *stream);

int icon_query_points_batch(const icon_mesh_batch_t *mb, const icon_feat_t *feat, const icon_mlp_t *mlp,
                            int prior_type, float sdf_clip, int cmap_mode, const float *d_calibs,
                            const float *d_points, int64_t N, int B, float *d_occ,
                            int search, int precision, icon_work_t *work, void *stream);

int icon_grid_eval_slab(const icon_mesh_t *mesh, const icon_feat_t *feat, const icon_mlp_t *mlp,
                        int prior_type, float sdf_clip, int cmap_mode,
                        int res, int z0, int z1, float *d_occ,
                        int search, int precision, icon_work_t *work, void *stream);

int icon_grid_slab_features(const icon_mesh_t *mesh, const icon_feat_t *feat,
                            int prior_type, float sdf_clip, int cmap_mode,
                            int res, int z0, int z1, int8_t *d_signs_local, int64_t *d_count_local,
                            int search, icon_work_t *work, void *stream);
int icon_grid_slab_finish(const icon_mlp_t *mlp, int res, int z0, int z1,
                          const int8_t *d_signs_global, int64_t k_total, int64_t rank_offset,
                          float *d_occ, int precision, icon_work_t *work, void *stream);
int icon_grid_slab_features_msg(const icon_mesh_t *mesh, const icon_feat_t *feat,
                                int prior_type, float sdf_clip, int cmap_mode,
                                int res, int z0, int z1, void *d_msg, int64_t msg_bytes,
                                int search, icon_work_t *work, void *stream);
int icon_grid_slab_finish_gathered(const icon_mlp_t *mlp, int res, int z0, int z1, int za, int zb,
                                   const void *d_gathered, int64_t stride, int world, int rank,
                                   float *d_occ, int precision, icon_work_t *work, void *stream);

int icon_adaptive_eval(const icon_mesh_t *mesh, const icon_feat_t *feat, const icon_mlp_t *mlp, int prior_type, float sdf_clip,
                       int cmap_mode, const int *resolutions, int n_levels, float balance, float *d_out, int64_t *h_counts,
                       int search, int precision, icon_work_t *work, void *stream);
int icon_adaptive_counts(icon_work_t *work, int n_levels, int64_t *h_counts, void *stream);
int icon_adaptive_reruns(icon_work_t *work, int *n);

int icon_query_rows(const icon_mesh_t *mesh, const icon_feat_t *feat, int prior_type, float sdf_clip, int cmap_mode,
                    const float *h_calib, const float *d_calib, const float *d_points, int64_t N, float *d_rows,
                    int search, icon_work_t *work, void *stream);
int icon_grid_rows(const icon_mesh_t *mesh, const icon_feat_t *feat, int prior_type, float sdf_clip, int cmap_mode,
                   int res, int z0, int z1, float *d_rows, int search, icon_work_t *work, void *stream);

int icon_debug_set_unfused(int on);
int icon_debug_mlp_pack_f16x3(int c0, const float *const *h_W, const float *const *h_b, uint16_t *img, float *side,
                              float *inv, float *scales);
int icon_debug_set_mesh_build(int host);
int icon_debug_mesh_layout(int64_t V, int64_t F, int64_t out[12]);
int icon_debug_host_mesh_build(const float *h_verts, int64_t V, const int64_t *h_faces, int64_t F,
                               const float *h_cmap, const float *h_vis, void *h_arena, int64_t arena_bytes);
int icon_debug_set_shell_skip(int on);
int icon_debug_set_option(const char *key, int value);
int icon_work_status(icon_work_t *work);

int icon_sdf_query_ties(const icon_mesh_t *mesh, const float *d_points, int64_t N,
                        int32_t *d_face, int32_t *d_face2, uint8_t *d_ulps, void *stream);
int icon_work_set_tie_rule(icon_work_t *work, int rule, int ulps);

int icon_debug_traversal_stats(const icon_mesh_t *mesh, int res, int z0, int z1, uint64_t out[4]);
int icon_debug_pair_stats(const icon_mesh_t *mesh, int res, int z0, int z1, uint64_t out[4]);
int icon_debug_walk_stats(const icon_mesh_t *mesh, int res, int z0, int z1, uint64_t out[6]);
int icon_debug_pair_box(const float *corners, int64_t n_pairs, const float *pts, int64_t n_pts, int shared_pts,
                        float *rec, int32_t *kind, float *bound);
int icon_debug_range_box(const float *tris, int64_t n_tris, float *rec, int32_t *kind);
int icon_debug_box_bound(const float *recs, int64_t n_recs, const float *pts, int64_t n_pts, int shared_pts, float *bound);
int icon_debug_box_bound_half(const float *recs, int64_t n_recs, const float *pts, int64_t n_pts, int shared_pts, float *bound);

int icon_volume_any_above(const float *d_occ, int res, int sx, int sy, int sz, float level, icon_work_t *work, void *stream, int *h_any);

int icon_export_mesh(const float *h_occ, int res, float level,
                     float *h_verts, int64_t *n_verts, int64_t *h_faces, int64_t *n_faces);

int icon_mc_count(const float *d_occ, int res, float level, icon_work_t *work, void *stream,
                  int64_t *n_verts, int64_t *n_faces);
int icon_mc_emit(float *d_verts, int64_t *d_faces, icon_work_t *work, void *stream);
int icon_mc_count_range(const float *d_occ, int res, float level, int zc0, int zc1, int halo, icon_work_t *work, void *stream,
                        int64_t *n_verts, int64_t *n_faces);
int icon_mc_emit_keyed(float *d_verts, int64_t *d_faces, int64_t *d_keys, icon_work_t *work, void *stream);

int icon_semantic_voxelize(const float *d_verts, int64_t V, int64_t V_surf, const float *d_code,
                           const int64_t *d_tets, int64_t T, int res, float sigma, float *d_out, void *stream);

int icon_semantic_voxelize_batch(const float *d_verts, int B, int64_t V, int64_t V_surf, const float *d_code,
                                 const int64_t *d_tets, int64_t T, int res, float sigma, uint8_t *d_occ, float *d_out, void *stream);

int icon_mesh_components(const int64_t *d_faces, int64_t F, int64_t V, int32_t *d_labels, void *stream);

int icon_clean_mesh(const float *d_verts, int64_t V, const int64_t *d_faces, int64_t F, float *d_out_verts, int32_t *d_out_faces,
                    int64_t *h_counts, icon_work_t *work, void *stream);

int icon_visibility(const float *d_xy, const float *d_z, int64_t V, const int64_t *d_faces, int64_t F,
                    int image_size, float *d_vis, void *stream);

int icon_query_color_bytes(int64_t V, int64_t F, int image_size, int64_t *bytes);
int icon_query_color(const float *d_verts, int64_t V, const void *d_faces, int64_t F, int faces_int64,
                     const float *d_image, int H, int W, int image_size, float *d_colors, float *d_vis,
                     void *d_scratch, int64_t scratch_bytes, void *stream);

int icon_render_bytes(int64_t V, int64_t F, int size, int n_views, int64_t *bytes);
int icon_render_normal(const float *d_verts, int64_t V, const void *d_faces, int64_t F, int faces_int64,
                       const int *cam_ids, int n_views, int size, float *d_images, float *d_depth, int32_t *d_pix_to_face,
                       void *d_scratch, int64_t scratch_bytes, void *stream);

int icon_silhouette_bytes(int64_t V, int64_t F, int size, int n_views, int64_t *bytes);
int icon_silhouette_forward(const float *d_verts, int64_t V, const void *d_faces, int64_t F, int faces_int64,
                            const int *cam_ids, int n_views, int size, float *d_alpha,
                            void *d_scratch, int64_t scratch_bytes, void *stream);
int icon_silhouette_backward(const float *d_verts, int64_t V, const void *d_faces, int64_t F, int faces_int64,
                             const int *cam_ids, int n_views, int size, const float *d_alpha, const float *d_grad_alpha,
                             float *d_grad_verts, void *d_scratch, int64_t scratch_bytes, void *stream);

int icon_render_normal_backward_bytes(int64_t V, int64_t F, int size, int n_views, int64_t *bytes);
int icon_render_normal_backward(const float *d_verts, int64_t V, const void *d_faces, int64_t F, int faces_int64,
                                const int *cam_ids, int n_views, int size, const int32_t *d_pix_to_face,
                                const float *d_grad_images, float *d_grad_verts,
                                void *d_scratch, int64_t scratch_bytes, void *stream);

int icon_render_turntable_bytes(int64_t V, int64_t F, int size, int n_views, int64_t *bytes);
int icon_render_turntable(const float *d_verts, int64_t V, const void *d_faces, int64_t F, int faces_int64,
                          const float *d_cos_sin, int n_views, int size, uint8_t *d_canvas, int64_t canvas_width, int64_t x0,
                          float *d_images, float *d_depth, int32_t *d_pix_to_face,
                          void *d_scratch, int64_t scratch_bytes, void *stream);

enum { ICON_PRIOR_EDGE = 1, ICON_PRIOR_NC = 2, ICON_PRIOR_LAPLACIAN = 4 };
int icon_local_affine_bytes(int64_t B, int64_t V, int64_t E, int64_t *bytes);
int icon_local_affine_forward(const float *d_x, const float *d_A, const float *d_b, int64_t B, int64_t V,
                              const void *d_edges, int64_t E, int index_int64, float *d_y, float *d_stiffness,
                              float *d_rigid, void *d_scratch, int64_t scratch_bytes, void *stream);
int icon_local_affine_backward(const float *d_x, const float *d_A, const float *d_b, int64_t B, int64_t V,
                               const void *d_nbr_off, const void *d_nbr, int64_t E, int index_int64,
                               const float *d_grad_y, const float *d_grad_stiffness, const float *d_grad_rigid,
                               float *d_grad_A, float *d_grad_b, void *stream);
int icon_mesh_priors_bytes(int64_t V, int64_t E, int64_t P, int64_t *bytes);
int icon_mesh_priors_forward(const float *d_verts, int64_t V, const void *d_edges, const void *d_nbr_off, const void *d_nbr, int64_t E,
                             const void *d_pairs, int64_t P, int index_int64, float target_length, int terms,
                             float *d_edge, float *d_nc, float *d_laplacian, void *d_scratch, int64_t scratch_bytes, void *stream);
int icon_mesh_priors_backward(const float *d_verts, int64_t V, const void *d_edges, const void *d_nbr_off, const void *d_nbr, int64_t E,
                              const void *d_pairs, const void *d_inc_off, const void *d_inc, int64_t P, int index_int64,
                              float target_length, int terms, const float *d_grad_edge, const float *d_grad_nc,
                              const float *d_grad_laplacian, float *d_grad_verts, void *d_scratch, int64_t scratch_bytes, void *stream);

typedef struct icon_smpl_tables {
    const float *v_template, *shapedirs, *posedirs, *J_template, *J_shapedirs;
    const int32_t *parents, *skin_idx;
    const float *skin_w;
    int64_t V;
    int32_t J, NB, K, P;
} icon_smpl_tables;
int icon_smpl_bytes(int64_t B, int64_t V, int J, int NB, int K, int64_t *bytes);
int icon_smpl_forward(const icon_smpl_tables *tables, const float *d_betas, const float *d_rot_mats, int64_t B,
                      float *d_verts, float *d_joints, float *d_A, void *stream);
int icon_smpl_backward(const icon_smpl_tables *tables, const float *d_betas, const float *d_rot_mats, int64_t B,
                       const float *d_A, const float *d_grad_verts, const float *d_grad_joints,
                       float *d_grad_betas, float *d_grad_rot_mats, void *d_scratch, int64_t scratch_bytes, void *stream);

int icon_nearest_vertex(const float *d_verts, int64_t V, const float *d_src, int64_t Vs, const uint8_t *d_only,
                        int32_t *d_out_idx, void *stream);
int icon_extract_cloth_bytes(int64_t V, int64_t F, int64_t total_poly_verts, int64_t P, int64_t *bytes);
int icon_extract_cloth(const float *d_verts, int64_t V, const void *d_faces, int64_t F, int faces_int64,
                       const double *d_poly_xy, const int32_t *d_poly_off, int64_t total_poly_verts, int64_t P,
                       const float *d_src, int64_t Vs, const uint8_t *d_src_remove,
                       float *d_out_verts, int32_t *d_out_faces, int32_t *d_out_vert_ids, int64_t *h_counts,
                       void *d_scratch, int64_t scratch_bytes, void *stream);

int icon_normal_consistency_bytes(int64_t Va, int64_t Fa, int64_t Vb, int64_t Fb, int size, int n_views, int64_t *bytes);
int icon_normal_consistency(const float *d_verts_a, int64_t Va, const void *d_faces_a, int64_t Fa, int faces_a_int64,
                            const float *d_normals_a, const float *d_verts_b, int64_t Vb, const void *d_faces_b, int64_t Fb,
                            int faces_b_int64, const float *d_normals_b, const float *d_view_mats, const float *d_view_muls,
                            int n_views, int size, double *d_err, float *d_rgba_a, float *d_rgba_b, int32_t *d_pix_a,
                            int32_t *d_pix_b, float *d_normals_out_a, float *d_normals_out_b, void *d_scratch,
                            int64_t scratch_bytes, void *stream);

int icon_sample_geo_bytes(int64_t n, int64_t *bytes);
int icon_sample_geo(const icon_mesh_t *scan, const float *d_verts, const float *d_vert_normals,
                    const double *calib, const double *calib_inv, int64_t N, double sigma_geo, int zray, int R,
                    uint64_t seed, float *d_samples, float *d_labels, int32_t *d_counts,
                    float *d_all_samples, uint8_t *d_all_inside, int32_t *d_all_source, int32_t *d_all_vertex,
                    void *d_scratch, int64_t scratch_bytes, void *stream);

int icon_train_rows_bytes(int B, int64_t N, int S, int C, int H, int W, int64_t *bytes);
int icon_train_rows_forward(const icon_mesh_batch_t *mb, int prior_type, float sdf_clip, int cmap_mode, int has_vis,
                            int has_cmap, int has_norm, const float *const *d_stacks, const int32_t *stack_shapes, int S,
                            const float *d_calibs, const float *d_points, int64_t N, float *d_rows, float *d_in_cube,
                            void *d_taps, int search, icon_work_t *work, void *stream);
int icon_train_rows_backward(const float *d_grad_rows, const void *d_taps, int S, uint32_t stack_mask, int B, int Cin, int C,
                             int H, int W, int n_select, int64_t N, float *d_grad_planes, void *d_scratch,
                             int64_t scratch_bytes, void *stream);

int icon_train_pamir_forward(const float *const *d_stacks, const int32_t *stack_shapes, const float *const *d_vols,
                             const int32_t *vol_shapes, int S, const float *d_calibs, const float *d_points, int64_t N,
                             float *d_rows, float *d_in_cube, void *d_taps, void *stream);
int icon_train_vol_bytes(int B, int64_t N, int S, int Cv, int D, int H, int W, int64_t *bytes);
int icon_train_vol_backward(const float *d_grad_rows, const void *d_taps, int S, uint32_t stack_mask, int B, int Cin, int C,
                            int Cv, int D, int H, int W, int64_t N, float *d_grad_vols, void *d_scratch,
                            int64_t scratch_bytes, void *stream);

#ifdef __cplusplus
}
#endif
#endif
```

Baseline: 1.165 billion.

## Fold shell zeroing, fast lattice decode and chunk totals into the sign pass

Adds a tail variant of the lattice sign kernel. It decodes indices with magic-number division and uses the precomputed LatticeFast world mapping. It also writes zeros to boundary-shell outputs directly, which lets the separate shell-fill kernel be skipped. It accumulates per-1024-block chunk totals with atomics, so the outlier list for large grids becomes a single chunked-scan launch instead of a multi-pass scan. The trade is extra atomics, a memset when the list state is dirty, and more state to track (list_dirty, shell_done). Debug peek and decode entry points are also added.

```diff
diff --git a/icon_amd/_lib.py b/icon_amd/_lib.py
--- a/icon_amd/_lib.py
+++ b/icon_amd/_lib.py
@@ -25,6 +25,7 @@
     "icon_volume_any_above", "icon_adaptive_eval", "icon_adaptive_counts", "icon_adaptive_reruns", "icon_grid_eval_slab", "icon_grid_slab_features", "icon_grid_slab_finish", "icon_grid_slab_features_msg",
     "icon_grid_slab_finish_gathered", "icon_debug_set_shell_skip", "icon_debug_set_option", "icon_work_status", "icon_sdf_query_ties", "icon_work_set_tie_rule",
     "icon_export_mesh", "icon_mc_count", "icon_mc_emit", "icon_mc_count_range", "icon_mc_emit_keyed", "icon_debug_traversal_stats", "icon_debug_pair_stats", "icon_debug_walk_stats", "icon_debug_pair_box", "icon_debug_range_box", "icon_debug_box_bound", "icon_debug_box_bound_half", "icon_debug_set_unfused", "icon_debug_mlp_pack_f16x3",
+    "icon_debug_work_peek", "icon_debug_lattice_decode",
     "icon_visibility", "icon_mesh_components", "icon_clean_mesh", "icon_semantic_voxelize",
     "icon_mesh_batch_create", "icon_mesh_batch_destroy", "icon_mesh_batch_status", "icon_feat_create_batch", "icon_query_points_batch",
     "icon_feat_batch_set_volume", "icon_semantic_voxelize_batch",
diff --git a/icon_amd/csrc/common.h b/icon_amd/csrc/common.h
--- a/icon_amd/csrc/common.h
+++ b/icon_amd/csrc/common.h
@@ -322,7 +322,8 @@
 int ensure_work(icon_work *w, int64_t n_points, bool need_x);
 void mark(icon_work *w, int k, hipStream_t st);
 bool want_fused(int precision, int search);
-int outlier_list(icon_work *w, int64_t N, const int *n_dev, int8_t *signs, bool counted, hipStream_t st);
+enum { kListUncounted = 0, kListCounted = 1, kListChunked = 2 };
+int outlier_list(icon_work *w, int64_t N, const int *n_dev, int8_t *signs, int counted, hipStream_t st);
 SignSrc self_signs(const icon_work *work, bool needs);
 int resolve_signs(const icon_work *work, SignSrc *sg, hipStream_t st);
 int outlier_patch(icon_work *w, int64_t N, int cmap_slot, const SignSrc &sg, hipStream_t st);
@@ -341,7 +342,7 @@
 extern int g_tt_chunk;
 extern int g_ev_lanes;
 enum Opt { kOptPairBox, kOptNodeBox, kOptBoxClamp, kOptLatticeFast, kOptUnfused, kOptShellSkip, kOptMcClassify1, kOptShareWaves, kOptShareRing, kOptShareLose,
-           kOptShareSpinLog2, kOptCount };
+           kOptShareSpinLog2, kOptGeomTail, kOptCount };
 int option(Opt o);
 }
 
@@ -364,6 +365,8 @@
     int64_t N = 0;
     const int32_t *map = nullptr;
     const int *n_dev = nullptr;
+    float *shell_out = nullptr;
+    bool shell_done = false;
     int c0 = 0;
     int cmap_slot = 0;
     bool needs_patch = false;
@@ -401,6 +404,8 @@
     int64_t *d_block_offsets = nullptr;
     int32_t *d_scan_local = nullptr;
     int64_t *d_scan_part = nullptr;
+    int32_t *d_chunk_tot = nullptr;
+    mutable bool list_dirty = true;
     int64_t cap_blocks = 0;
     int8_t *d_signs = nullptr;
     int64_t cap_signs = 0;
@@ -413,6 +418,7 @@
     int64_t cap_rows = 0;
     int *h_err = nullptr;
     icon::LatticeFast *d_lfast = nullptr;
+    const icon::LatticeFast *lfast_call = nullptr;
     uint32_t *d_sort_keys = nullptr;
     int32_t *d_sort_idx = nullptr;
     void *d_sort_tmp = nullptr;
@@ -448,4 +454,12 @@
     r.map = c.map;
     return r;
 }
-}
+inline bool sign_tail(const QueryCall &c, const icon_work *w)
+{
+    return c.src == Src::Lattice && !c.n_dev && c.N <= 0xffffffffll && w->lfast_call != nullptr && option(kOptGeomTail) != 0;
+}
+inline bool sign_leaves_chunks(const QueryCall &c, const icon_work *w)
+{
+    return sign_tail(c, w) && c.needs_patch && (c.N + kScanBlock - 1) / kScanBlock > 1024;
+}
+}
diff --git a/icon_amd/csrc/fused_f16x3.hip b/icon_amd/csrc/fused_f16x3.hip
--- a/icon_amd/csrc/fused_f16x3.hip
+++ b/icon_amd/csrc/fused_f16x3.hip
@@ -73,13 +73,19 @@
     rec[1] = __builtin_amdgcn_s_memrealtime();
 }
 
+struct SignTail {
+    uint32_t res_magic;
+    const LatticeFast *lf;
+    float *shell_out;
+    int32_t *chunk_tot;
+};
 static_assert(kScanBlock == 256, "k_sign's 256-point blocks are the blocks of the outlier scan and the tiles of the fused kernel");
-template <bool LATTICE>
+template <bool LATTICE, bool TAIL = false>
 __global__ __launch_bounds__(256) void k_sign(MeshDev m, Calib cal, int res, int z0, const float *__restrict__ pts, int64_t N,
                                               float sdf_clip, const int32_t *__restrict__ row_count, const int32_t *__restrict__ row_slots,
                                               NearRef near, uint8_t *__restrict__ code8,
                                               int32_t *__restrict__ block_counts, unsigned long long *__restrict__ grp_mask, float far_box2,
-                                              const int *__restrict__ n_dev, int *__restrict__ range_flag)
+                                              const int *__restrict__ n_dev, int *__restrict__ range_flag, SignTail t)
 {
     __shared__ int wsum[4];
     if (range_flag && blockIdx.x == 0 && threadIdx.x == 0) *range_flag = 0;
@@ -89,7 +95,14 @@
     uint32_t code = 0;
     if (live) {
     f3 p; bool ins;
-    if (LATTICE) {
+    if (LATTICE && TAIL) {
+        int ix, iy, iz;
+        const int64_t row = (int64_t)lattice_decode32((uint32_t)i, (uint32_t)res, t.res_magic, ix, iy, iz);
+        p = lattice_world_fast(t.lf, ix, iy, iz + z0);
+        ins = inside_row(m, p, row_count, row_slots, row);
+        const int e = res - 1;
+        if (t.shell_out && (ix == 0 || ix == e || iy == 0 || iy == e || iz + z0 == 0 || iz + z0 == e)) t.shell_out[i] = 0.0f;
+    } else if (LATTICE) {
         const int64_t row = i / res;
         const int ix = (int)(i - row * res), iy = (int)(row % res), iz = (int)(row / res);
         p = lattice_world(res, ix, iy, iz + z0);
@@ -109,7 +122,11 @@
         grp_mask[(int64_t)blockIdx.x * 4 + (threadIdx.x >> 6)] = b;
     }
     __syncthreads();
-    if (threadIdx.x == 0) block_counts[blockIdx.x] = wsum[0] + wsum[1] + wsum[2] + wsum[3];
+    if (threadIdx.x == 0) {
+        const int s = wsum[0] + wsum[1] + wsum[2] + wsum[3];
+        block_counts[blockIdx.x] = s;
+        if (TAIL && t.chunk_tot && s) atomicAdd(t.chunk_tot + (blockIdx.x >> 10), s);
+    }
 }
 
 template <bool BATCH>
@@ -470,9 +487,23 @@
     ICON_ARG(nb > 0 && nb < (1ll << 31), "too many workgroups for one launch");
     const float far_box2 = far_box_dist2(c.sdf_clip);
     const NearRef near = work_near(work, c);
-    if (c.src == Src::Lattice) hipLaunchKernelGGL(k_sign<true>, dim3((unsigned)nb), dim3(256), 0, st, c.mesh->dev, c.cal, c.L.res, c.L.z0, c.points, N, c.sdf_clip,
+    if (sign_tail(c, work)) {
+        SignTail t{};
+        t.res_magic = udiv_magic((uint32_t)c.L.res);
+        t.lf = work->lfast_call;
+        t.shell_out = c.L.off ? c.shell_out : nullptr;
+        if (sign_leaves_chunks(c, work)) {
+            if (work->list_dirty) ICON_HIP(hipMemsetAsync(work->d_chunk_tot, 0, (size_t)(1 + (work->cap_blocks + 1023) / 1024) * sizeof(int32_t), st));
+            work->list_dirty = true;
+            t.chunk_tot = work->d_chunk_tot + 1;
+        }
+        hipLaunchKernelGGL((k_sign<true, true>), dim3((unsigned)nb), dim3(256), 0, st, c.mesh->dev, c.cal, c.L.res, c.L.z0, c.points, N, c.sdf_clip,
+                           work->d_row_count, work->d_row_slots, near, work->d_code8, work->d_block_counts,
+                           (unsigned long long *)work->d_grp_mask, far_box2, (const int *)nullptr, work->d_flag, t);
+    }
+    else if (c.src == Src::Lattice) hipLaunchKernelGGL(k_sign<true>, dim3((unsigned)nb), dim3(256), 0, st, c.mesh->dev, c.cal, c.L.res, c.L.z0, c.points, N, c.sdf_clip,
                                                   work->d_row_count, work->d_row_slots, near, work->d_code8, work->d_block_counts,
-                                                  (unsigned long long *)work->d_grp_mask, far_box2, (const int *)nullptr, work->d_flag);
+                                                  (unsigned long long *)work->d_grp_mask, far_box2, (const int *)nullptr, work->d_flag, SignTail{});
     else if (c.src == Src::Batch)
         hipLaunchKernelGGL(k_sign_wide<true>, dim3((unsigned)nb), dim3(1024), 0, st, MeshDev{}, Calib{}, c.points, N, c.sdf_clip, near, work->d_code8,
                            work->d_block_counts, (unsigned long long *)work->d_grp_mask, far_box2, (const int *)nullptr, work->d_flag, c.bd);
@@ -481,7 +512,7 @@
                            work->d_block_counts, (unsigned long long *)work->d_grp_mask, far_box2, c.n_dev, work->d_flag, BatchDev{});
     else hipLaunchKernelGGL(k_sign<false>, dim3((unsigned)nb), dim3(256), 0, st, c.mesh->dev, c.cal, c.L.res, c.L.z0, c.points, N, c.sdf_clip,
                             (const int32_t *)nullptr, (const int32_t *)nullptr, near, work->d_code8, work->d_block_counts,
-                            (unsigned long long *)work->d_grp_mask, far_box2, c.n_dev, work->d_flag);
+                            (unsigned long long *)work->d_grp_mask, far_box2, c.n_dev, work->d_flag, SignTail{});
     ICON_HIP(hipGetLastError());
     work->flag_clean = work->d_flag != nullptr;
     return ICON_OK;
@@ -535,7 +566,7 @@
     G.f = c.feat->dev; G.cal = c.cal; G.pts = c.points; G.sdf_clip = c.sdf_clip; G.cmap_local = c.cmap_mode == ICON_CMAP_LOCAL ? 1 : 0;
     if (lattice) {
         const int zs = std::max(za, L.off), ze = std::min(zb, L.res - L.off);
-        if (L.off) {
+        if (L.off && !(c.shell_done && c.shell_out == d_occ)) {
             const int64_t rows = (int64_t)(zb - za) * L.res;
             const int row_wgs = (int)((rows + 255) / 256);
             const int64_t face_rows = 2 * (int64_t)(zb - za) + (int64_t)((za == 0 ? 1 : 0) + (zb == L.res ? 1 : 0)) * L.res;
@@ -615,3 +646,15 @@
 }
 
 }
+
+extern "C" int icon_debug_lattice_decode(int res, int64_t i0, int64_t n, int64_t *out)
+{
+    ICON_ARG(res >= 1 && i0 >= 0 && n >= 0 && i0 + n <= 0x100000000ll && out != nullptr, "icon_debug_lattice_decode: bad argument");
+    const uint32_t m = icon::udiv_magic((uint32_t)res);
+    for (int64_t k = 0; k < n; ++k) {
+        int ix, iy, iz;
+        const uint32_t row = icon::lattice_decode32((uint32_t)(i0 + k), (uint32_t)res, m, ix, iy, iz);
+        out[4 * k] = ix; out[4 * k + 1] = iy; out[4 * k + 2] = iz; out[4 * k + 3] = (int64_t)row;
+    }
+    return ICON_OK;
+}
diff --git a/icon_amd/csrc/geom_device.h b/icon_amd/csrc/geom_device.h
--- a/icon_amd/csrc/geom_device.h
+++ b/icon_amd/csrc/geom_device.h
@@ -906,10 +906,20 @@
 constexpr int kLatticeFastMaxRes = 2048;
 constexpr size_t kLatticeFastBytes = sizeof(LatticeFast) + kLatticeFastMaxRes * sizeof(float);
 __host__ __device__ inline uint32_t udiv_magic(uint32_t d) { return d > 1 ? (uint32_t)(0x100000000ull / d) : 0xffffffffu; }
-__device__ __forceinline__ uint32_t udiv_fast(uint32_t n, uint32_t d, uint32_t m)
-{
+__host__ __device__ __forceinline__ uint32_t udiv_fast(uint32_t n, uint32_t d, uint32_t m)
+{
+#if defined(__HIP_DEVICE_COMPILE__)
     const uint32_t q = __umulhi(n, m);
+#else
+    const uint32_t q = (uint32_t)(((uint64_t)n * m) >> 32);
+#endif
     return q + ((n - q * d >= d) ? 1u : 0u);
+}
+__host__ __device__ __forceinline__ uint32_t lattice_decode32(uint32_t i, uint32_t res, uint32_t m, int &ix, int &iy, int &iz)
+{
+    const uint32_t row = udiv_fast(i, res, m), z = udiv_fast(row, res, m);
+    ix = (int)(i - row * res); iy = (int)(row - z * res); iz = (int)z;
+    return row;
 }
 __device__ __forceinline__ void lattice_fast_write(LatticeFast *out, LatticeMap L, const MeshDev &m)
 {
diff --git a/icon_amd/csrc/outlier_list.hip b/icon_amd/csrc/outlier_list.hip
--- a/icon_amd/csrc/outlier_list.hip
+++ b/icon_amd/csrc/outlier_list.hip
@@ -105,6 +105,40 @@
     for (int k = 0; k < w; ++k) r += wsum[k];
     if (o) signs[r] = (int8_t)code_sign(code);
 }
+__global__ __launch_bounds__(kScanBlock) void k_outlier_chunked(const int32_t *__restrict__ counts, int32_t *chunk_tot, int nchunks,
+                                                                const uint8_t *__restrict__ code8, int64_t N, int64_t *__restrict__ block_offsets,
+                                                                int64_t *__restrict__ total, int8_t *__restrict__ signs)
+{
+    __shared__ int wsum[kScanBlock / 64];
+    __shared__ int64_t red[2][kScanBlock / 64];
+    const int chunk = (int)(blockIdx.x >> 10);
+    const bool want_all = blockIdx.x == 0;
+    int64_t before = 0, all = 0;
+    for (int k = threadIdx.x; k < (want_all ? nchunks : chunk); k += kScanBlock) {
+        const int64_t t = __hip_atomic_load(chunk_tot + 1 + k, __ATOMIC_RELAXED, __HIP_MEMORY_SCOPE_AGENT);
+        all += t; if (k < chunk) before += t;
+    }
+    for (int64_t k = ((int64_t)chunk << 10) + threadIdx.x; k < (int64_t)blockIdx.x; k += kScanBlock) before += counts[k];
+    for (int d = 32; d >= 1; d >>= 1) { before += __shfl_xor(before, d); all += __shfl_xor(all, d); }
+    const int lane = threadIdx.x & 63, w = threadIdx.x >> 6;
+    const int64_t i = (int64_t)blockIdx.x * kScanBlock + threadIdx.x;
+    const uint32_t code = (i < N) ? code8[i] : 0u;
+    const bool o = code & kCodeOutlier;
+    const unsigned long long b = __ballot(o);
+    if (lane == 0) { red[0][w] = before; red[1][w] = all; wsum[w] = __popcll(b); }
+    __syncthreads();
+    before = 0; all = 0;
+    for (int k = 0; k < kScanBlock / 64; ++k) { before += red[0][k]; all += red[1][k]; }
+    if (threadIdx.x == 0) {
+        block_offsets[blockIdx.x] = before;
+        if (want_all) *total = all;
+        if (atomicAdd(chunk_tot, 1) == (int)gridDim.x - 1)
+            for (int k = 0; k <= nchunks; ++k) atomicExch(chunk_tot + k, 0);
+    }
+    int64_t r = before + __popcll(b & ((1ull << lane) - 1ull));
+    for (int k = 0; k < w; ++k) r += wsum[k];
+    if (o) signs[r] = (int8_t)code_sign(code);
+}
 constexpr int64_t kSmallListBlocks = 16384;
 
 __global__ __launch_bounds__(kScanBlock) void k_outlier_patch(float *__restrict__ X, const uint8_t *__restrict__ code8, int64_t N, int cmap_slot,
@@ -146,11 +180,20 @@
     seg[world] = a;
 }
 
-int outlier_list(icon_work *w, int64_t N, const int *n_dev, int8_t *signs, bool counted, hipStream_t st)
+int outlier_list(icon_work *w, int64_t N, const int *n_dev, int8_t *signs, int counted, hipStream_t st)
 {
     const int64_t nblk = (N + kScanBlock - 1) / kScanBlock;
-    if (!counted) hipLaunchKernelGGL(k_outlier_count, dim3((unsigned)nblk), dim3(kScanBlock), 0, st, w->d_code8, N, w->d_block_counts);
+    if (counted == kListUncounted) hipLaunchKernelGGL(k_outlier_count, dim3((unsigned)nblk), dim3(kScanBlock), 0, st, w->d_code8, N, w->d_block_counts);
     const bool one = nblk <= (n_dev ? kSmallListBlocks : 1024);
+    if (counted == kListChunked) {
+        ICON_ARG(!n_dev && nblk > 0 && nblk <= w->cap_blocks, "outlier list: chunk totals without a host-side size");
+        hipLaunchKernelGGL(k_outlier_chunked, dim3((unsigned)nblk), dim3(kScanBlock), 0, st, w->d_block_counts, w->d_chunk_tot, (int)((nblk + 1023) / 1024),
+                           w->d_code8, N, w->d_block_offsets, w->d_total, signs);
+        ICON_HIP(hipGetLastError());
+        w->list_dirty = false;
+        debug_sync("outlier list (one launch behind the sign pass)", st);
+        return ICON_OK;
+    }
     if (one) {
         hipLaunchKernelGGL(k_outlier_small, dim3((unsigned)std::max<int64_t>(nblk, 1)), dim3(kScanBlock), 0, st, w->d_block_counts, w->d_code8, N, w->d_block_offsets, w->d_total,
                            signs, n_dev);
diff --git a/icon_amd/csrc/query_kernels.hip b/icon_amd/csrc/query_kernels.hip
--- a/icon_amd/csrc/query_kernels.hip
+++ b/icon_amd/csrc/query_kernels.hip
@@ -312,6 +312,7 @@
             if (!work->d_lfast) ICON_HIP(hipMalloc((void **)&work->d_lfast, kLatticeFastBytes));
             lf = work->d_lfast;
         }
+        work->lfast_call = lf;
         if (rows <= 20000)
             hipLaunchKernelGGL(k_row_crossings_wide, dim3((unsigned)((rows * 16 + kBlock - 1) / kBlock)), dim3(kBlock), 0, st, mesh->dev, L,
                                work->d_row_count, work->d_row_slots, lf);
@@ -380,7 +381,7 @@
     int rc;
     if ((rc = launch_sign(c, work, st))) return rc;
     if (!c.n_dev) debug_sync(c.src == Src::Batch ? "k_sign_wide<batch>" : "k_sign", st);
-    if (c.needs_patch && (rc = outlier_list(work, c.N, c.n_dev, d_signs_out ? d_signs_out : work->d_signs, true, st))) return rc;
+    if (c.needs_patch && (rc = outlier_list(work, c.N, c.n_dev, d_signs_out ? d_signs_out : work->d_signs, sign_leaves_chunks(c, work) ? kListChunked : kListCounted, st))) return rc;
     return ICON_OK;
 }
 
@@ -390,11 +391,13 @@
     if (c.prior != ICON_PRIOR_ICON) return ICON_OK;
     if (c.search == ICON_SEARCH_BRUTE) {
         if ((rc = feature_rows(c, work, st))) return rc;
-        return c.needs_patch ? outlier_list(work, c.N, nullptr, d_signs_out ? d_signs_out : work->d_signs, false, st) : ICON_OK;
+        return c.needs_patch ? outlier_list(work, c.N, nullptr, d_signs_out ? d_signs_out : work->d_signs, kListUncounted, st) : ICON_OK;
     }
     rc = c.src == Src::Points ? launch_nearest<false>(c, work, st) : c.src == Src::Lattice ? launch_nearest<true>(c, work, st) : launch_nearest_batch(c, work, st);
     if (rc) return rc;
-    return sign_and_list(c, d_signs_out, work, st);
+    if ((rc = sign_and_list(c, d_signs_out, work, st))) return rc;
+    c.shell_done = sign_tail(c, work) && c.L.off && c.shell_out != nullptr;
+    return ICON_OK;
 }
 
 int call_finish(QueryCall &c, const icon_mlp *mlp, const SignSrc &fs, float *d_occ, int precision, icon_work *work, hipStream_t st, int za, int zb)
@@ -492,11 +495,11 @@
 
 static int slab_features_impl(const icon_mesh_t *mesh, const icon_feat_t *feat, int prior_type, float sdf_clip, int cmap_mode,
                               int res, int z0, int z1, int8_t *d_signs_local, int64_t *d_count_local, void *d_msg, int64_t msg_bytes,
-                              int search, icon_work_t *work, void *stream)
+                              int search, icon_work_t *work, void *stream, float *shell_out = nullptr)
 {
     ICON_ARG(work != nullptr, "icon_grid_slab_features: work is null");
     QueryCall c = query_call("icon_grid_slab_features", Src::Lattice, feat, prior_type, sdf_clip, cmap_mode, search);
-    c.mesh = mesh;
+    c.mesh = mesh; c.shell_out = shell_out;
     int rc = describe_call(c);
     if (rc) return rc;
     if ((rc = lattice_map(res, z0, z1, prior_type == ICON_PRIOR_ICON ? mesh : nullptr, sdf_clip, search != ICON_SEARCH_BRUTE, &c.L))) return rc;
@@ -674,7 +677,8 @@
                                    int search, int precision, icon_work_t *work, void *stream)
 {
     ICON_ARG(mlp && work && d_occ, "icon_grid_eval_slab: null argument");
-    int rc = icon_grid_slab_features(mesh, feat, prior_type, sdf_clip, cmap_mode, res, z0, z1, nullptr, nullptr, search, work, stream);
+    int rc = slab_features_impl(mesh, feat, prior_type, sdf_clip, cmap_mode, res, z0, z1, nullptr, nullptr, nullptr, 0, search, work, stream,
+                                want_fused(precision, search) ? d_occ : nullptr);
     if (rc) return rc;
     QueryCall &c = work->slab;
     ICON_ARG(c.c0 == mlp->c0, "icon_grid_eval_slab: MLP input width does not match the feature layout");
diff --git a/icon_amd/csrc/work.hip b/icon_amd/csrc/work.hip
--- a/icon_amd/csrc/work.hip
+++ b/icon_amd/csrc/work.hip
@@ -20,6 +20,7 @@
      [](int v) { return v >= 0; }, "a ticket >= 1, or 0"},
     {kOptShareSpinLog2, "share_spin_log2", nullptr, 0,
      [](int v) { return v >= 0 && v < 30; }, "0..29"},
+    {kOptGeomTail, "geometry_tail", "ICON_AMD_GEOMETRY_TAIL", 1},
 };
 constexpr bool options_in_enum_order(int o = 0) { return o == kOptCount || (kOptions[o].id == o && options_in_enum_order(o + 1)); }
 static_assert(options_in_enum_order(), "kOptions[] must list the switches in the order of enum Opt");
@@ -98,6 +99,9 @@
         ICON_HIP(hipMalloc((void **)&w->d_block_offsets, (size_t)nblk * sizeof(int64_t)));
         ICON_HIP(hipMalloc((void **)&w->d_scan_local, (size_t)nblk * sizeof(int32_t)));
         ICON_HIP(hipMalloc((void **)&w->d_scan_part, (size_t)((nblk + 1023) / 1024) * sizeof(int64_t)));
+        (void)hipFree(w->d_chunk_tot); w->d_chunk_tot = nullptr;
+        ICON_HIP(hipMalloc((void **)&w->d_chunk_tot, (size_t)(1 + (nblk + 1023) / 1024) * sizeof(int32_t)));
+        w->list_dirty = true;
         w->cap_blocks = nblk;
     }
     if (n_points > w->cap_signs) {
@@ -125,6 +129,7 @@
         w->cap_points_hi = w->cap_points;
     }
     w->slab_ready = false;
+    w->lfast_call = nullptr;
     return ICON_OK;
 }
 
@@ -157,7 +162,7 @@
     (void)hipFree(w->d_signs); (void)hipFree(w->d_total); (void)hipFree(w->d_flag); (void)hipFree(w->d_seg); (void)hipFree(w->d_row_count); (void)hipFree(w->d_row_slots); (void)hipFree(w->d_lfast); if (w->h_err) (void)hipHostFree(w->h_err); if (w->h_any) (void)hipHostFree(w->h_any); (void)hipFree(w->d_near16); (void)hipFree(w->d_near_hi); (void)hipFree(w->d_near_d2); (void)hipFree(w->d_code8);
     (void)hipFree(w->d_sort_keys); (void)hipFree(w->d_sort_idx); (void)hipFree(w->d_sort_tmp);
     for (int k = 0; k < 6; ++k) if (w->ev[k]) (void)hipEventDestroy(w->ev[k]);
-    (void)hipFree(w->d_clock); (void)hipFree(w->d_steal);
+    (void)hipFree(w->d_clock); (void)hipFree(w->d_steal); (void)hipFree(w->d_chunk_tot);
     icon::mc_destroy(w->mc);
     icon::clean_destroy(w->clean);
     icon::adaptive_destroy(w->ad);
@@ -300,6 +305,22 @@
     return ICON_OK;
 }
 
+extern "C" int icon_debug_work_peek(icon_work_t *w, int what, void *dst, int64_t n, void *stream)
+{
+    ICON_ARG(w != nullptr && dst != nullptr && n >= 0, "icon_debug_work_peek: bad argument");
+    const void *src = nullptr;
+    size_t bytes = 0;
+    if (what == 0) { ICON_ARG(n <= w->cap_points, "icon_debug_work_peek: more code bytes than the workspace holds"); src = w->d_code8; bytes = (size_t)n; }
+    else if (what == 1) { ICON_ARG(n <= w->cap_blocks, "icon_debug_work_peek: more blocks than the workspace holds"); src = w->d_block_offsets; bytes = (size_t)n * sizeof(int64_t); }
+    else if (what == 2) { ICON_ARG(n == 1, "icon_debug_work_peek: the total is one word"); src = w->d_total; bytes = sizeof(int64_t); }
+    else if (what == 3) { ICON_ARG(n <= w->cap_signs, "icon_debug_work_peek: more signs than the workspace holds"); src = w->d_signs; bytes = (size_t)n; }
+    else return fail(ICON_ERR_ARG, "icon_debug_work_peek: what must be 0..3");
+    if (bytes == 0) return ICON_OK;
+    ICON_ARG(src != nullptr, "icon_debug_work_peek: no call has run on this workspace");
+    ICON_HIP(hipMemcpyAsync(dst, src, bytes, hipMemcpyDefault, (hipStream_t)stream));
+    return ICON_OK;
+}
+
 extern "C" int icon_debug_set_unfused(int on)
 {
     set_option(kOptUnfused, on);
diff --git a/icon_amd/engine.py b/icon_amd/engine.py
--- a/icon_amd/engine.py
+++ b/icon_amd/engine.py
@@ -341,6 +341,15 @@
         n = C.c_int(0)
         check(_lib.lib().icon_adaptive_reruns(self.h, C.byref(n)), "icon_adaptive_reruns")
         return int(n.value)
+
+    def peek(self, what: str, n: int, device) -> torch.Tensor:
+        kinds = {"code8": (0, torch.uint8), "block_offsets": (1, torch.int64), "total": (2, torch.int64), "signs": (3, torch.int8)}
+        k, dtype = kinds[what]
+        out = torch.empty(int(n), dtype=dtype, device=device)
+        if out.numel() == 0:
+            return out
+        check(_lib.lib().icon_debug_work_peek(self.h, C.c_int(k), ptr(out), C.c_int64(int(n)), _stream()), "icon_debug_work_peek")
+        return out
 
     def stage_ms(self):
         out = (C.c_float * 3)()
diff --git a/include/icon_amd.h b/include/icon_amd.h
--- a/include/icon_amd.h
+++ b/include/icon_amd.h
@@ -142,6 +142,8 @@
                                const float *h_cmap, const float *h_vis, void *h_arena, int64_t arena_bytes);
 int icon_debug_set_shell_skip(int on);
 int icon_debug_set_option(const char *key, int value);
+int icon_debug_work_peek(icon_work_t *work, int what, void *dst, int64_t n, void *stream);
+int icon_debug_lattice_decode(int res, int64_t i0, int64_t n, int64_t *out);
 int icon_work_status(icon_work_t *work);
 
 int icon_sdf_query_ties(const icon_mesh_t *mesh, const float *d_points, int64_t N,
```

Result: slower. 912.3 million (-21.7%).
